# jiaxiZeng/Temporally-Consistent-Stereo-Matching

Hardware: AMD Instinct MI355X
Metric: stereo-pairs/sec at 640x480 D=192, 32 GRU iters (higher is better)
Workload: dtype f32

## Files before the change

### include/tcs_mi355.h

```cpp
#ifndef TCS_MI355_H
#define TCS_MI355_H

#include <stddef.h>
#include <stdint.h>

#ifdef __cplusplus
extern "C" {
#endif

#define TCS_OK 0
#define TCS_EINVAL (-1)
#define TCS_ELAUNCH (-2)
#define TCS_EUNSUPPORTED (-3)

typedef void* tcs_stream_t;

int tcs_abi_version(void);
const char* tcs_error_string(int code);


size_t tcs_corr_level_bytes(int B, int H, int W, int level);
size_t tcs_corr_build_workspace_bytes(int B, int H, int W);

int tcs_corr_build(const float* fmap1, const float* fmap2, int B, int C, int H, int W,
// ... 85 lines not shown
                      int B, int H, int W, float* refined, float* delta_disp, float* coords1, float* flow_x, float* flow_x_ch,
                      long long flow_x_ch_bstride, tcs_stream_t stream);

int tcs_convex_upsample(const float* disp, const float* mask, int B, int H, int W, int clip, float* flow_up, float* flow_q,
                        tcs_stream_t stream);

int tcs_convex_upsample_pair(const float* disp_a, const float* disp_b, const float* mask, int B, int H, int W, float* up_a, float* up_b,
                             float* q_a, float* q_b, tcs_stream_t stream);

int tcs_avgpool3s2(const float* x, int B, int C, int H, int W, float* out, tcs_stream_t stream);

int tcs_resize_bilinear(const float* x, int B, int C, int H, int W, int Ho, int Wo, float* out, tcs_stream_t stream);
int tcs_resize_bilinear_scaled(const float* x, int B, int C, int H, int W, int Ho, int Wo, float scale, float* out, tcs_stream_t stream);

#define TCS_ACT_NONE 0
#define TCS_ACT_RELU 1
#define TCS_ACT_SIGMOID 2
#define TCS_ACT_TANH 3
#define TCS_ACT_LEAKY 4
#define TCS_ACT_RELU_ADD_RELU 5

#define TCS_EPI_LINEAR 0
#define TCS_EPI_GRU_ZR 1
#define TCS_EPI_GRU_Q 2
#define TCS_EPI_BLEND9 4
#define TCS_EPI_DECONV2X 3

#define TCS_MATH_F32 0
#define TCS_MATH_F16X3 1

#define TCS_MAX_SRC 4

typedef struct tcs_conv_desc {
    const float* src[TCS_MAX_SRC];
    int src_ch[TCS_MAX_SRC];
    int n_src;
    const float* weight;
    const float* bias;
    int B, H, W;
    int Cin, Cout, ksize;
    int epilogue;
    int act;
    float post_scale;
    const float* addend;
    const float* addend2;
    const float* h;
    const float* z;
    int blend_keep_z;
    float* out;
    int out_ctot, out_coff;
    float* out2;
    int stride;
    int math;
    float weight_unscale;
    void* out16;
    int out16_groups, out16_group_offset;
    int in_transform;
    const float* src_batch2;
    int batch_split;
    int products;
} tcs_conv_desc;

size_t tcs_conv_packed_floats(int Cout, int Cin, int ksize);
int tcs_pack_conv_weight(const float* w_oihw, int Cout, int Cin, int ksize, float* packed, tcs_stream_t stream);
size_t tcs_conv_packed_floats_f16x3(int Cout, int Cin, int ksize);
int tcs_pack_conv_weight_f16x3(const float* w_oihw, int Cout, int Cin, int ksize, int scale_log2, float* packed,
                               tcs_stream_t stream);
size_t tcs_deconv_packed_floats_f16x3(int Cin, int Cout);
int tcs_pack_deconv4x4s2_f16x3(const float* w_iohw, int Cin, int Cout, int scale_log2, float* packed, float* scratch_oihw,
                               tcs_stream_t stream);
int tcs_instance_norm(const float* x, int B, int C, int H, int W, float eps, int act, const float* addend, float* out,
                      tcs_stream_t stream);
int tcs_conv3x3_cout1(const float* x, const float* w_oihw, const float* bias, int B, int Cin, int H, int W, float* out,
                      tcs_stream_t stream);
int tcs_conv2d(const tcs_conv_desc* desc, tcs_stream_t stream);
int tcs_conv2d_group(const tcs_conv_desc* const* descs, int n, tcs_stream_t stream);
int tcs_conv2d_group_fused(const tcs_conv_desc* const* descs, int n);

size_t tcs_s16_bytes(int B, int C, int H, int W);
int tcs_s16_flags(unsigned int* flags_out);
#define TCS_S16_FLAG_UNITS 5
int tcs_s16_flags_detail(unsigned int* per_unit);
int tcs_s16_from_f32(const float* x, int B, int C, int H, int W, void* s16, int groups_total, int group_offset, tcs_stream_t stream);
int tcs_s16_to_f32(const void* s16, int B, int C, int H, int W, int groups_total, int group_offset, float* out, tcs_stream_t stream);

typedef struct tcs_conv_s16_desc {
    const void* src[TCS_MAX_SRC];
    int src_ch[TCS_MAX_SRC];
    int src_groups[TCS_MAX_SRC];
    int n_src;
    const float* weight;
    const float* bias;
    int B, H, W;
    int Cin, Cout, ksize;
    int stride;
    int epilogue;
    int act;
    float post_scale;
    float weight_unscale;
    const float* addend;
    const float* addend2;
    const void* addend16;
    int addend16_groups;
    const void* h;
    int h_groups;
    const float* z;
    int blend_keep_z;
    void* out16;
    int out16_groups, out16_group_offset;
    float* out32;
    int out_ctot, out_coff;
    int tile_cfg;
    int addend_ctot;
    const float* blend_cand;
    int blend_cand_ctot;
    const float* blend_disp;
    float* blend_refined;
    float* blend_delta;
    float* blend_coords1;
    float* blend_flow_x;
    void* blend_flow16;
    int blend_flow16_groups, blend_flow16_channel;
    void* out16b;
    int out16b_groups, out16_split;
    void* in_stats;
    float in_eps;
    const float* tap_weights;
    float* tap_out;
    int tap_nout, tap_tiles;
    float tap_unscale;
    const float* blend_warm_pyr[4];
    int blend_warm_radius;
    int products;
} tcs_conv_s16_desc;

int tcs_avgpool3s2_s16(const void* x, int B, int groups, int H, int W, void* out, int out_groups, tcs_stream_t stream);
int tcs_resize_bilinear_s16(const void* x, int B, int groups, int H, int W, int Ho, int Wo, void* out, int out_groups, tcs_stream_t stream);
size_t tcs_instance_norm_s16_workspace_bytes(int B, int groups, int H, int W);
int tcs_instance_norm_s16(const void* x, int B, int groups, int H, int W, float eps, int act, const void* addend, int addend_groups,
                          void* out, int out_groups, void* workspace, tcs_stream_t stream);
size_t tcs_deconv_in_stats_bytes(int B, int C, int H_in, int W_in);
int tcs_instance_norm_apply_s16(const void* x, int B, int groups, int H, int W, int act, const void* addend, int addend_groups,
                                void* out, int out_groups, const void* in_stats, int C, float eps, tcs_stream_t stream);
size_t tcs_tap_weights_floats(int nout, int C);
int tcs_pack_tap_weights(const float* w_oihw, int nout, int C, int scale_log2, float* packed, tcs_stream_t stream);
int tcs_taps_sum(const float* taps, int ntile, int nout, const float* bias, const float* addend, float scale, int B, int H, int W, float* out,
                 tcs_stream_t stream);
int tcs_flow_taps_step_grads(const float* coords1, const float* taps, int ntile, const float* bias, int B, int H, int W, float scale,
                             float* disp_q, float* grad, float* cands, float* delta_out, tcs_stream_t stream);
int tcs_taps_propagate_s16(const float* taps, int ntile, const float* bias2, const float* g5, float post_scale, const float* disp, int B, int H,
                           int W, float* grad_out, float* cand9, void* out16, int out_groups, tcs_stream_t stream);
int tcs_propagate_disparity_s16(const float* grad, const float* disp, int B, int H, int W, float* cand9, void* out16, int out_groups,
                                tcs_stream_t stream);
int tcs_s16_set_channel(const float* x, int B, int H, int W, void* s16, int groups_total, int channel, tcs_stream_t stream);
int tcs_softmax_blend_s16(const float* logits9, const float* cand, int cand_ctot, const float* disp_q,
                          int B, int H, int W, float* refined, float* delta_disp, float* coords1, float* flow_x,
                          void* flow_x_s16, int flow_x_s16_groups, int flow_x_s16_channel, tcs_stream_t stream);

size_t tcs_weight_frags_bytes(int Cout, int Cin);
int tcs_pack_weight_frags(const float* w_oi, int Cout, int Cin, int natural_channels, int scale_log2, void* packed, tcs_stream_t stream);
int tcs_hidden_update_s16(void* h, int h_groups, const float* delta, const float* w1, const float* b1, const void* W2, const float* b2,
                          float unscale2, const void* Wzr, const float* bzr, float unscale_zr, const void* Wq, const float* bq,
                          float unscale_q, int B, int H, int W, tcs_stream_t stream);

int tcs_conv2d_s16(const tcs_conv_s16_desc* desc, tcs_stream_t stream);

int tcs_conv2d_s16_group(const tcs_conv_s16_desc* const* descs, int n, tcs_stream_t stream);
int tcs_conv2d_s16_group_fused(const tcs_conv_s16_desc* const* descs, int n);

typedef struct tcs_s16_instance { int ksize, stride, epilogue, mt, rows, ksteps, nstage, row_split, rows_per_wave, taps,
                                  products, csplit, blocks, threads; long long lds_bytes; } tcs_s16_instance;
int tcs_conv2d_s16_plan(const tcs_conv_s16_desc* desc, tcs_s16_instance* out);

#define TCS_LOSS_MAX_ITERS 64
#define TCS_LOSS_SEQ 1
#define TCS_LOSS_INIT 2
#define TCS_LOSS_GRAD 4
#define TCS_LOSS_NORM 8
#define TCS_LOSS_OUT_TOTAL 0
#define TCS_LOSS_OUT_SEQ 1
#define TCS_LOSS_OUT_INIT 2
#define TCS_LOSS_OUT_NORM 3
#define TCS_LOSS_OUT_GRAD 4
#define TCS_LOSS_OUT_EPE 5
#define TCS_LOSS_OUT_INIT_GT 14
#define TCS_LOSS_OUT_INIT_NM 15
#define TCS_LOSS_OUT_FMR 16
#define TCS_LOSS_OUT_FLAGS 17
#define TCS_LOSS_NOUT 18

size_t tcs_loss_workspace_bytes(int B, int H, int W, int iters);
int tcs_loss_targets(const float* flow_gt, const void* valid, int valid_mode, int B, int H, int W, float* grad_gt, float* norm_gt,
                     uint8_t* grad_mask, uint8_t* norm_mask, uint8_t* valid_dense, uint8_t* valid_sparse, tcs_stream_t stream);
int tcs_loss_targets_full(const float* gt, int C, const void* valid, int valid_mode, int B, int H, int W, float* out, uint8_t* gt_mask,
                          uint8_t* valid_dense, uint8_t* valid_sparse, tcs_stream_t stream);
int tcs_sequence_loss(const float* preds, long long iter_stride, long long refine_offset, int iters, const float* flow_gt,
                      const void* valid, int valid_mode, const float* flow_mono, const float* flow_init, int B, int H, int W,
                      double* workspace, tcs_stream_t stream);
int tcs_init_loss(const float* cost_volume, int D, const float* flow_gt, const void* valid, int valid_mode, int B, int H, int W, int k,
                  float threshold, int iters, double* workspace, tcs_stream_t stream);
int tcs_grad_normal_loss(const float* grad_preds, long long grad_stride, const float* q_preds, long long q_stride, long long q_refine_offset,
                         int iters, const float* grad_gt, const uint8_t* grad_mask, const uint8_t* grad_valid, const float* norm_gt,
                         const uint8_t* norm_mask, const uint8_t* norm_valid, int B, int H, int W, double* workspace, tcs_stream_t stream);
int tcs_loss_finish(const double* workspace, int parts, int B, int H, int W, int iters, int k, const double* loss_weights, double* out,
                    float* out32, tcs_stream_t stream);

#define TCS_LOSS_COUNT_SEQ 0
#define TCS_LOSS_COUNT_INIT 1
#define TCS_LOSS_COUNT_NORM 2
#define TCS_LOSS_COUNT_GRAD 3
#define TCS_LOSS_NCOUNTS 4
int tcs_loss_finish_counts(const double* workspace, int parts, int B, int H, int W, int iters, int k, const double* loss_weights,
                           double* out, float* out32, double* counts, tcs_stream_t stream);
int tcs_sequence_loss_bwd(const float* preds, long long iter_stride, long long refine_offset, int iters, const float* flow_gt,
                          const void* valid, int valid_mode, const float* flow_mono, const float* flow_init, int B, int H, int W,
                          const double* loss_weights, const double* counts, const float* upstream, float* grad_preds, float* grad_mono,
                          float* grad_init, tcs_stream_t stream);
int tcs_init_loss_bwd(const float* cost_volume, int D, const float* flow_gt, const void* valid, int valid_mode, int B, int H, int W, int k,
                      float threshold, const double* counts, const float* upstream, float* grad_cost_volume, tcs_stream_t stream);
int tcs_grad_normal_loss_bwd(const float* grad_preds, long long grad_stride, const float* q_preds, long long q_stride,
                             long long q_refine_offset, int iters, const float* grad_gt, const uint8_t* grad_mask, const uint8_t* grad_valid,
                             const float* norm_gt, const uint8_t* norm_mask, const uint8_t* norm_valid, int B, int H, int W,
                             const double* loss_weights, const double* counts, const float* upstream, float* grad_grad_preds,
                             float* grad_q_preds, tcs_stream_t stream);

int tcs_upsample_flow(const float* flow, const float* mask, int B, int H, int W, float* flow_up, tcs_stream_t stream);
int tcs_upsample_flow_pair(const float* flow_a, const float* flow_b, const float* mask, int B, int H, int W, float* up_a, float* up_b,
                           tcs_stream_t stream);
size_t tcs_convex_upsample_backward_workspace_floats(int B, int H, int W, int n_flows);
int tcs_convex_upsample_backward(const float* flow, const float* mask, const float* grad_up, int B, int H, int W, float* grad_mask,
                                 float* grad_flow, float* workspace, tcs_stream_t stream);
int tcs_convex_upsample_pair_backward(const float* flow_b, const float* mask, const float* grad_up_a, const float* grad_up_b, int B, int H,
                                      int W, float* grad_mask, float* grad_flow_a, float* grad_flow_b, float* workspace, tcs_stream_t stream);
int tcs_refine_blend(const float* logits9, const float* disp_grads, const float* disp, int B, int H, int W, float* refined,
                     tcs_stream_t stream);
int tcs_refine_blend_backward(const float* logits9, const float* disp_grads, const float* disp, const float* grad_refined, int B, int H,
                              int W, float* grad_logits, float* grad_disp_grads, tcs_stream_t stream);

#ifdef __cplusplus
}
#endif
#endif
```

### temporally-consistent-stereo-matching_amd/core/tc_stereo.py

```python
import contextlib
import os

import torch
import torch.nn as nn

from core.corr import CorrBlock1D
from core.extractor import BasicEncoder, MultiBasicEncoder, ResidualBlock, hip_head
from core.update import (IN_SUM_SLOTS, BasicMultiUpdateBlock, DispGradPredictor, DispRefine, DisparityCompletor, HiddenstateUpdater,
                         Lightfuse, hip_conv)
from core.utils.utils import coords_grid
from tcs_mi355 import ops, s16


class autocast(contextlib.AbstractContextManager):

    def __init__(self, enabled=False, **_):
        self.enabled = enabled

    def __exit__(self, *exc):
        return False


HIP_PRECISIONS = {"fp32": 0, "fp16": 1}

# ... 144 lines not shown
        if test_mode:
            return self._pipeline()(image1, image2, iters, temporal, use_graph=self._graph_mode())
        out = self._pipeline()(image1, image2, iters, temporal, use_graph=self._graph_mode(), outputs=True)
        return self._training_output(out, iters)

    @staticmethod
    def _training_output(out, iters):
        up, q, grad = out["up"], out["q"], out["grad"]
        return {"flow_mono": out["flow_mono"], "flow_init": out["flow_init"],
                "flow_predictions": [[up[k, 0], up[k, 1]] for k in range(iters)],
                "flow_q_predictions": [[q[k, 0], q[k, 1]] for k in range(iters)],
                "disp_grad_q_predictions": [grad[k] for k in range(iters)],
                "cost_volume": out["cost_volume"],
                "flow_q": out["flow_q"], "net_list": out["net_list"], "fmap1": out["fmap1"]}

    def _frame(self, image1, image2, iters, temporal, outputs=False):
        feats = self._extract_stage(image1, image2, temporal is None or len(temporal) == 8, outputs)
        return self._refine_loop(feats, self._refine_head(feats, temporal), iters, outputs)

    def _extract_stage(self, image1, image2, first, cost_volume=False):
        a = self.args

        def correlate(fmap1, fmap2):
            corr_fn = CorrBlock1D(fmap1, fmap2, radius=a.corr_radius, num_levels=a.corr_levels, thres=a.init_thres, want_argmax=first,
                                  want_cost_volume=cost_volume)
            return corr_fn, (corr_fn.argmax_disp() if first else None)

        def context(cnet_list, relu_done=False):
            inp = [x[1] if relu_done else torch.relu(x[1]) for x in cnet_list]
            grads = [hip_conv(conv, [i]) for i, conv in zip(inp, self.context_zqr_convs_grad)]
            zqr = [list(hip_conv(conv, [i]).chunk(3, 1)) for i, conv in zip(inp, self.context_zqr_convs)]
            return zqr, grads, [x[0] for x in cnet_list]

        if a.shared_backbone and self.cnet.can16(image1):
            from tcs_mi355.streams import fork_join
            trunk = self.cnet.trunk16(image1, right=image2, raw_images=True)

            def matching_side():
                fm = hip_head(self.conv2, trunk)
                f1, f2 = (t.float().contiguous() for t in fm.split(fm.shape[0] // 2, 0))
                return f1, f2, correlate(f1, f2)

            (fmap1, fmap2, (corr_fn, prior)), (inp_list, grad_list, net_list) = fork_join(
                [matching_side, lambda: context(self.cnet.heads16(trunk, True, a.n_gru_layers, relu_context=True), relu_done=True)])
        else:
            image1 = (2 * (image1 / 255.0) - 1.0).contiguous()
            image2 = (2 * (image2 / 255.0) - 1.0).contiguous()
            cnet_list, fmap1, fmap2 = self._features(image1, image2)
            corr_fn, prior = correlate(fmap1, fmap2)
            inp_list, grad_list, net_list = context(cnet_list)
        return {"fmap1": fmap1, "corr_fn": corr_fn, "prior": prior, "inp_list": inp_list, "grad_list": grad_list, "net_list": net_list}

    def _refine_head(self, feats, temporal):
        first = temporal is None
        start = temporal[7] if temporal is not None and len(temporal) == 8 else None
        fmap1, corr_fn = feats["fmap1"], feats["corr_fn"]
        net_list = feats["net_list"]
        if first:
            last_net_list = None
            sparse_disp, cost, sparse_mask = feats["prior"] if feats["prior"] is not None else corr_fn.argmax_disp()
        else:
            K, T, previous_T, baseline, last_disp, last_net_list, last_fmap1 = temporal[:7]
            K_scale, K_scale_inv, relative_T, back_T = ops.pose_prepare(K, T, previous_T, self.scale_rate, start=start)
            prior = None if start is None else (feats["prior"] if feats["prior"] is not None else corr_fn.argmax_disp())
            sparse_disp, _, sparse_mask, cost = ops.warp_forward(
                (-last_disp).float().contiguous(), last_fmap1.float().contiguous(), relative_T, K_scale,
                K_scale_inv, baseline, cur_fmap=fmap1, want_fmap=False, ordered=self._hip_deterministic, start=start, prior=prior)

        pool = self._s16pool
        disp_init, disp_mono, _, net_list = self.disp_completor.run16(pool, sparse_disp, cost, sparse_mask,
                                                                      [c.float().contiguous() for c in net_list], tanh_nets=True)
        disp_init = disp_init.float().contiguous()

        if last_net_list is None:
            warped = None
        else:
            grid = ops.backward_grid(disp_init, back_T, K_scale, K_scale_inv, baseline)
            warped = []
            for i, net in enumerate(last_net_list):
                warped.append(ops.bilinear_sample(net.float().contiguous(), grid, start=start))
                if i + 1 < len(last_net_list):
                    grid = ops.grid_halve(grid)

        for i, (h, fuse) in enumerate(zip(net_list, self.previous_current_hideen_fuse)):
            if warped is None:
                x = pool.get(("frame", "zero", i), h.B, h.C, h.H, h.W, h.device)
            else:
                x = s16.to_s16(warped[i], out=pool.get(("frame", "warped", i), h.B, h.C, h.H, h.W, h.device))
            fuse.step16(pool, h, [x])

        coords0 = self._coords0(fmap1)
        coords1 = (coords0 - disp_init).contiguous()
        trace = getattr(self, "_trace", None)
        if trace is not None:
            trace.update(sparse_disp=sparse_disp, cost=cost, sparse_mask=sparse_mask, disp_init=disp_init,
                         net0=[t.float().clone() for t in net_list], iters=[])
        return {"coords1": coords1, "net_list": net_list, "disp_init": disp_init, "disp_mono": disp_mono}

    def _refine_loop(self, feats, start, iters, outputs=False):
        a = self.args
        fmap1, corr_fn = feats["fmap1"], feats["corr_fn"]
        inp_list, grad_list = feats["inp_list"], feats["grad_list"]
        coords1, nets = start["coords1"], start["net_list"]
        coords0 = self._coords0(fmap1)
        trace = getattr(self, "_trace", None)

        pool = self._s16pool
        n3 = a.n_gru_layers == 3
        grads16 = [s16.to_s16(t.float().contiguous(), out=pool.get(("frame", "ctxg", i), t.shape[0], t.shape[1], t.shape[2], t.shape[3], t.device))
                   for i, t in enumerate(grad_list)]
        dg_pre = self.disp_grad_refine.prepare(pool, grads16)
        self.disp_grad_refine.begin_frame(pool, coords1.shape[0], coords1.device)
        refined = up_mask = None
        flows_x = (coords1 - coords0).contiguous()
        motion = pool.get(("frame", "motion"), coords1.shape[0], 128, coords1.shape[2], coords1.shape[3], coords1.device)
        s16.set_channel(flows_x, motion, 127)
        ub = self.update_block
        ub.begin_frame()
        from tcs_mi355.streams import fork_join, join, mark, spawn
        hu_delta = None
        early32 = None
        plain = not a.slow_fast_gru and n3
        side = _OutputsSide(self, pool, coords1, iters, start) if outputs else None
        for itr in range(iters):
            def enc_branch():
                corr = corr_fn(coords1)
                return corr, ub.encoder.run(pool, flows_x, corr, motion)

            def coarse_branch():
                if hu_delta is not None:
                    self.hiddenstate_update.run(pool, nets[0], hu_delta)
                if up32_now is not None:
                    return ub.gru16_late(pool, nets, up32_now[1])
                if n3 and a.slow_fast_gru:
                    ub.run_coarse(pool, nets, inp_list, iter16=False, iter32=True, want_up16=False)
                if a.n_gru_layers >= 2 and a.slow_fast_gru:
                    ub.run_coarse(pool, nets, inp_list, iter16=True, iter32=n3, want_up16=False)
                return ub.run_coarse(pool, nets, inp_list, iter16=a.n_gru_layers >= 2, iter32=n3, up32=up32_now)

            up32_now = join(early32)
            early32 = None
            up16, (corr, m) = fork_join([coarse_branch, enc_branch])
            if side is not None:
                side.launch()
            run_ahead = plain and trace is None and itr + 1 < iters
            def ahead():
                up32 = ub.run_gru32(pool, nets, inp_list)
                return up32, ub.gru16_early(pool, nets, inp_list, up32)
            at_join = mark() if run_ahead else None
            sums = getattr(self, "_checksums", None)
            lazy = trace is None and sums is None
            delta_flow = ub.run_fine(pool, nets, inp_list, m, up16, lazy=lazy)
            if at_join is not None:
                early32 = spawn(ahead, after=at_join)
            if isinstance(delta_flow, s16.Taps):
                disp_q, g5, cands = s16.flow_taps_step_grads(coords1, delta_flow, scale=5.0)
            else:
                disp_q, g5, cands = ops.flow_step_grads(coords1, delta_flow, scale=5.0)
            disp_grad, context = self.disp_grad_refine.run(pool, g5, cands, dg_pre, lazy=lazy, slot=itr if itr < IN_SUM_SLOTS else None)
            last = itr == iters - 1
            warm = corr_fn._pyr if (not last and a.corr_levels == 4) else None
            if side is None:
                refined, up_mask, fused = self.disp_refine.run(pool, disp_grad, disp_q, nets[0], context, want_mask=last, motion=motion,
                                                               warm_pyramid=warm, warm_radius=a.corr_radius)
            else:
                refined, up_mask, fused = self.disp_refine.run(pool, disp_grad, disp_q, nets[0], context, motion=motion,
                                                               warm_pyramid=warm, warm_radius=a.corr_radius, grad_out=side.grad[itr],
                                                               before_fuse=side.join)
                side.record(itr, disp_q, refined, fused["fused"])
            hu_delta = fused["delta_disp"]
            coords1, flows_x = fused["coords1"], fused["flow_x"]
            if sums is not None:
                sums.append({k: v.double().sum() for k, v in dict(
                    corr=corr, motion=m.data, net0=nets[0].data, net1=nets[1].data, net2=nets[2].data, delta_flow=delta_flow,
                    disp_grad=disp_grad, context=context.data, refined=refined, coords1=coords1).items()})
            if trace is not None:
                self.hiddenstate_update.run(pool, nets[0], hu_delta)
                hu_delta = None
                trace["iters"].append(dict(corr=corr, delta=delta_flow, disp_q=disp_q, refined=refined,
                                           net=[t.float() for t in nets]))
        if hu_delta is not None:
            self.hiddenstate_update.run(pool, nets[0], hu_delta)
        if side is not None:
            side.launch()
            up_mask = side.join()
        net_list = [t.float() for t in nets]

        flow_up, flow_q = ops.convex_upsample(refined.contiguous(), up_mask)
        out = {"flow": flow_up, "flow_q": flow_q, "net_list": [x.detach() for x in net_list], "fmap1": fmap1.detach()}
        if side is not None:
            out.update(side.outputs(corr_fn))
        return out

# ... 52 lines not shown
```

### temporally-consistent-stereo-matching_amd/core/update.py

```python
import torch
import torch.nn as nn
import torch.nn.functional as F

from core.utils.basic_layers import Conv2x_IN
from tcs_mi355 import ops, s16
from tcs_mi355.streams import fork_join


CONV_MATH = "f16x3"


def products_of(conv: nn.Module) -> int:
    if getattr(conv, "_tcs_x3", False):
        return 0
    pool = getattr(conv, "_s16pool", None)
    return 0 if pool is None else pool.products


def packed(conv: nn.Conv2d) -> ops.PackedConv:
    w, b = conv.weight, conv.bias
    math = getattr(conv, "_tcs_math", None) or CONV_MATH
    if conv.stride == (2, 2):
        math = "f16x3"
    nprod = products_of(conv) if math == "f16x3" else 0
# ... 21 lines not shown


def packed16_part(conv: nn.Conv2d, cin_slices, with_bias: bool = True) -> ops.PackedConv:
    w, b = conv.weight, conv.bias
    nprod = products_of(conv)
    key = (w.data_ptr(), w._version, w.device, None if b is None else (b.data_ptr(), b._version), nprod)
    cache = conv.__dict__.setdefault("_tcs_parts", {})
    spec = (tuple(tuple(int(v) for v in sl) for sl in cin_slices), bool(with_bias))
    hit = cache.get(spec)
    if hit is None or hit[0] != key:
        ws = torch.cat([w.detach()[:, lo:hi] for lo, hi in spec[0]], 1).contiguous()
        hit = (key, ops.pack_conv(ws, b if with_bias else None, "f16x3", nprod))
        cache[spec] = hit
    return hit[1]


def packed16_cat(convs) -> ops.PackedConv:
    nprod = products_of(convs[0])
    key = tuple((c.weight.data_ptr(), c.weight._version, None if c.bias is None else (c.bias.data_ptr(), c.bias._version)) for c in convs) + (nprod,)
    host = convs[0]
    cache = host.__dict__.setdefault("_tcs_cat", {})
    ids = tuple(id(c) for c in convs)
    hit = cache.get(ids)
    if hit is None or hit[0] != key:
        w = torch.cat([c.weight.detach() for c in convs], 0).contiguous()
        b = torch.cat([(c.bias.detach() if c.bias is not None else torch.zeros(c.out_channels, device=c.weight.device)) for c in convs], 0).contiguous()
        hit = (key, ops.pack_conv(w, b, "f16x3", nprod))
        cache[ids] = hit
    return hit[1]


def tap_weights(conv2: nn.Conv2d) -> torch.Tensor:
    w = conv2.weight
    key = (w.data_ptr(), w._version, w.device)
    hit = getattr(conv2, "_tcs_taps", None)
    if hit is None or hit[0] != key:
        hit = (key, s16.pack_taps(w))
        conv2._tcs_taps = hit
    return hit[1]


def tap_partials(pool, conv1: nn.Conv2d, conv2: nn.Conv2d, srcs, pc=None, out16b=None) -> s16.Taps:
    a = srcs[0]
    ntile = (conv1.out_channels + 31) // 32
    taps = s16.Taps(pool.get32((id(conv2), "taps"), (a.B, ntile, 9 * conv2.out_channels, a.H, a.W), a.device), ntile, conv2.out_channels,
                    None if conv2.bias is None else conv2.bias.detach())
    s16.conv2d(packed16(conv1) if pc is None else pc, srcs, act="relu", taps=taps, tap_weights=tap_weights(conv2), out16b=out16b,
               out16_split=conv1.out_channels if out16b is not None else 0)
    return taps


def pool_of(module) -> s16.S16Pool:
    p = getattr(module, "_s16pool", None)
    if p is None:
        p = s16.S16Pool()
        for m in module.modules():
            m._s16pool = p
    return p


def conv16(pool, conv, srcs, act="none", addend=None, post_scale=1.0, out=None, want32=False, tag="o", addend16=None, pc=None, tile_cfg=0):
    a = srcs[0]
    pc = packed16(conv) if pc is None else pc
    stride = conv.stride[0]
    Ho, Wo = ((a.H - 1) // 2 + 1, (a.W - 1) // 2 + 1) if stride == 2 else (a.H, a.W)
    if want32:
        return s16.conv2d(pc, srcs, act=act, addend=addend, post_scale=post_scale, want32=True, stride=stride, addend16=addend16)[1]
    if out is None:
        out = pool.get((id(conv), tag), a.B, conv.out_channels, Ho, Wo, a.device)
    return s16.conv2d(pc, srcs, act=act, addend=addend, post_scale=post_scale, out16=out, stride=stride, addend16=addend16, tile_cfg=tile_cfg)[0]


def conv32to16(pool, conv, x, act="none", tag="o", image_pair=None, in_transform=0):
    B, _, H, W = (int(v) for v in x.shape)
    B += 0 if image_pair is None else int(image_pair.shape[0])
    out = pool.get((id(conv), tag), B, conv.out_channels, H, W, x.device)
    return ops.conv2d(packed(conv), [x.float().contiguous()], act=act, out16=out,
                      image_pair=None if image_pair is None else image_pair.float().contiguous(), in_transform=in_transform)


def to16(pool, x, key):
    B, C_, H, W = (int(v) for v in x.shape)
    return s16.to_s16(x.float().contiguous(), out=pool.get(key, B, C_, H, W, x.device))


IN_SUM_SLOTS = 64


def up_block16(pool, block: Conv2x_IN, x: s16.S16, rem: s16.S16, slot=None) -> s16.S16:
    dc = block.conv1.conv
    y = pool.get((id(dc), "o"), x.B, dc.out_channels, 2 * x.H, 2 * x.W, x.device)
    stats = None
    if slot is not None and s16.deconv_in_stats_ok(x.B, dc.out_channels, x.H, x.W):
        stats = up_block_sums(pool, block, x.B, x.device)[int(slot)]
    s16.deconv4x4s2(packed_deconv(dc), [x], out16=y, in_stats=stats)
    norm = (lambda **kw: s16.instance_norm_apply(y, stats, **kw)) if stats is not None else (lambda **kw: s16.instance_norm(y, **kw))
    if (y.H, y.W) != (rem.H, rem.W):
        y32 = F.interpolate(norm(act="leaky", out=y).float(), size=(rem.H, rem.W), mode="nearest") + rem.float()
        y = to16(pool, y32, (id(dc), "resized"))
    else:
        y = norm(act="leaky", addend=rem, out=y)
    act2 = "leaky" if block.conv2.relu else "none"
    if block.conv2.use_in:
        z = conv16(pool, block.conv2.conv, [y])
        return s16.instance_norm(z, act=act2, out=z)
    return conv16(pool, block.conv2.conv, [y], act=act2)


def up_block_sums(pool, block: Conv2x_IN, B: int, device) -> torch.Tensor:
    dc = block.conv1.conv
    stride = s16.nv.lib().tcs_deconv_in_stats_bytes(1, dc.out_channels, 8, 8) // (8 * dc.out_channels)
    return pool.get_i64((id(dc), "in_sums"), (IN_SUM_SLOTS, int(B), dc.out_channels, stride), device)


def hip_conv(conv, srcs, act="none", **kw):
    return ops.conv2d(packed(conv), [s.float().contiguous() for s in srcs], act=act, stride=conv.stride[0], **kw)


def packed_deconv(deconv: nn.ConvTranspose2d) -> ops.PackedConv:
    w = deconv.weight
    nprod = products_of(deconv)
    key = (w.data_ptr(), w._version, w.device, nprod)
    hit = getattr(deconv, "_tcs_packed", None)
    if hit is None or hit[0] != key:
        if deconv.kernel_size != (4, 4) or deconv.stride != (2, 2) or deconv.padding != (1, 1) or deconv.bias is not None:
            raise NotImplementedError(f"tcs deconv covers ConvTranspose2d(4, stride 2, pad 1, bias=False), got {deconv}")
        hit = (key, ops.pack_deconv4x4s2(w, nprod))
        deconv._tcs_packed = hit
    return hit[1]


def _conv(cin, cout, k, stride=1):
    return nn.Conv2d(cin, cout, k, stride, k // 2)


def _two(cin, mid, cout, k=3, tail=None):
    layers = [_conv(cin, mid, k), nn.ReLU(inplace=True), _conv(mid, cout, k)]
    return nn.Sequential(*layers, *([tail] if tail is not None else []))


class _GateCell(nn.Module):
    keep_z = False

    def __init__(self, hidden_dim, input_dim, kernel_size):
        super().__init__()
        self.convzr = _conv(hidden_dim + input_dim, hidden_dim * 2, kernel_size)
        self.convq = _conv(hidden_dim + input_dim, hidden_dim, kernel_size)

    def _step(self, h, xs, cz=None, cr=None, cq=None):
        h = h.float().contiguous()
        xs = [x.float().contiguous() for x in xs]
        z, rh = ops.gru_gates(packed(self.convzr), [h, *xs], h, cz, cr)
        return ops.gru_update(packed(self.convq), [rh, *xs], h, z, cq, keep_z=self.keep_z)

    def step16(self, pool, h: s16.S16, xs, cz=None, cr=None, cq=None) -> s16.S16:
        z = pool.get32((id(self), "z"), (h.B, h.C, h.H, h.W), h.device)
        rh = pool.get((id(self), "rh"), h.B, h.C, h.H, h.W, h.device)
        ctot = lambda t: 0 if (t is None or t.is_contiguous()) else int(t.stride(0)) // (h.H * h.W)
        if ctot(cz) != ctot(cr):
            cz, cr = cz.contiguous(), cr.contiguous()
        s16.gru_gates(packed16(self.convzr), [h, *xs], h, cz, cr, z_out=z, rh_out=rh, addend_ctot=ctot(cz))
        return s16.gru_update(packed16(self.convq), [rh, *xs], h, z, cq, keep_z=self.keep_z, out=h, addend_ctot=ctot(cq))


class ConvGRU(_GateCell):
    def __init__(self, hidden_dim, input_dim, kernel_size=3):
# ... 305 lines not shown

    def propagate_disparity(self, disparity_grad, disparity_map):
        buf = ops.propagate_disparity(disparity_grad.float().contiguous(), disparity_map.float().contiguous())
        return buf[:, :9], buf[:, 9:]

    def forward(self, disp_grads, disp, context_disp, context_grad, test_mode=False, fused_outputs=None):
        pool = pool_of(self)
        cd = to16(pool, context_disp, (id(self), "ctxd_in"))
        cg = to16(pool, context_grad, (id(self), "ctxg_in"))
        refined, mask, extra = self.run(pool, disp_grads.float().contiguous(), disp.float().contiguous(), cd, cg, want_mask=not test_mode)
        if fused_outputs is not None:
            fused_outputs.update({k: v for k, v in extra.items() if k != "fused"})
        return refined, mask

    def mask_head(self, pool, fused: s16.S16, out: torch.Tensor = None) -> torch.Tensor:
        m = conv16(pool, self.mask[0], [fused], act="relu")
        if out is None:
            return conv16(pool, self.mask[2], [m], post_scale=0.25, want32=True)
        return s16.conv2d(packed16(self.mask[2]), [m], post_scale=0.25, out32=out)[1]

    def run(self, pool, disp_grads: torch.Tensor, disp: torch.Tensor, context_disp: s16.S16, context_grad: s16.S16, want_mask=False,
            motion: s16.S16 = None, warm_pyramid=None, warm_radius: int = 4, grad_out: torch.Tensor = None, before_fuse=None):
        f27 = pool.get((id(self), "f27"), disp.shape[0], 27, disp.shape[2], disp.shape[3], disp.device)
        if isinstance(disp_grads, tuple):
            f27, cand9, self._last_grad = s16.taps_propagate(disp_grads[0], disp_grads[1], disp_grads[2], disp, out16=f27, grad=grad_out)
        else:
            f27, cand9 = s16.propagate_disparity(disp_grads, disp, out16=f27)
            if grad_out is not None:
                grad_out.copy_(disp_grads)

        cc, ds = self.context_compress, self.disp_f_stem
        t3 = 101411 if context_disp.H * context_disp.W >= 10000 else 0
        with s16.grouped():
            c = conv16(pool, cc[0], [context_disp, context_grad], act="relu", tile_cfg=t3)
            d = conv16(pool, ds[0], [f27], act="relu")
        with s16.grouped():
            context = conv16(pool, cc[2], [c], tile_cfg=t3)
            disp_f = conv16(pool, ds[2], [d])
        fused = conv16(pool, self.conv_fuse[0], [disp_f, context], act="relu")
        if before_fuse is not None:
            before_fuse()
        fused = conv16(pool, self.conv_fuse[2], [fused], act="relu")
        w = conv16(pool, self.w_head[0], [fused], act="relu")
        coords1, flow_x = torch.empty_like(disp), torch.empty_like(disp)
        refined, delta = s16.conv1x1_blend(packed16(self.w_head[2]), [w], cand9, disp, coords1, flow_x, flow_x_s16=motion,
                                           flow_x_channel=127, warm_pyramid=warm_pyramid, warm_radius=warm_radius)
        mask = self.mask_head(pool, fused) if want_mask else None
        return refined, mask, dict(delta_disp=delta, coords1=coords1, flow_x=flow_x, fused=fused)


class DisparityCompletor(nn.Module):
    def __init__(self):
        super().__init__()
        relu = lambda: nn.ReLU(inplace=True)
        mlp = lambda cin, mid, cout: nn.Sequential(_conv(cin, mid, 1), relu(), _conv(mid, cout, 1))
        cin_block = lambda cin, mid, cout, s=1: nn.Sequential(_conv(cin, mid, 3, s), nn.InstanceNorm2d(mid), relu(), _conv(mid, cout, 3))
        self.conv_disp_stem = mlp(1, 64, 64)
        self.conv_cost_stem = mlp(1, 32, 32)
        self.conv_mask_stem = mlp(1, 32, 32)
        self.conv_disp_fuse = mlp(128, 128, 64)
        self.conv_4_4 = cin_block(192, 192, 64)
        self.conv_4_8 = cin_block(64, 64, 64, 2)
        self.conv_8_8 = cin_block(192, 192, 64)
        self.conv_8_16 = cin_block(64, 64, 64, 2)
        self.conv_16_16 = cin_block(192, 192, 64)
        self.conv_16_8 = Conv2x_IN(64, 64, deconv=True, concat=False, keep_concat=False, IN=True)
        self.conv_8_4 = Conv2x_IN(64, 64, deconv=True, concat=False, keep_concat=False, IN=True)
        self.disp_head = _two(64, 128, 1)
        self.w_head = _two(64, 128, 1, tail=nn.Sigmoid())
        self.conv_out16_disp = cin_block(192, 192, 128)
        self.conv_out8_disp = cin_block(192, 192, 128)
        self.conv_out4_disp = cin_block(192, 192, 128)

    def run16(self, pool, disp, cost, mask, ctx, tanh_nets=False):
        d = (disp / 10).float().contiguous()

        def stem(seq, x):
            return conv16(pool, seq[2], [conv32to16(pool, seq[0], x.float().contiguous(), act="relu")])

        def cin(seq, srcs, act="none"):
            y = conv16(pool, seq[0], srcs)
            return conv16(pool, seq[3], [s16.instance_norm(y, act="relu", out=y)], act=act)

        c16 = [to16(pool, c, (id(self), "ctx", i)) for i, c in enumerate(ctx)]
        x4_disp = conv16(pool, self.conv_disp_fuse[2], [conv16(pool, self.conv_disp_fuse[0], [stem(self.conv_disp_stem, d),
                         stem(self.conv_cost_stem, cost), stem(self.conv_mask_stem, mask - 0.5)], act="relu")])
        x4 = cin(self.conv_4_4, [x4_disp, c16[0]])
        x8 = cin(self.conv_8_8, [cin(self.conv_4_8, [x4]), c16[1]])
        x16_out = cin(self.conv_16_16, [cin(self.conv_8_16, [x8]), c16[2]])
        x8_out = up_block16(pool, self.conv_16_8, x16_out, x8)
        x4_out = up_block16(pool, self.conv_8_4, x8_out, x4)
        disp_mono = conv16(pool, self.disp_head[2], [conv16(pool, self.disp_head[0], [x4_out], act="relu")], want32=True)
        w = conv16(pool, self.w_head[2], [conv16(pool, self.w_head[0], [x4_out], act="relu")], act="sigmoid", want32=True)
        completed = (w * d + (1 - w) * disp_mono) * 10
        na = "tanh" if tanh_nets else "none"
        nets = [cin(self.conv_out4_disp, [x4_out, c16[0]], na), cin(self.conv_out8_disp, [x8_out, c16[1]], na),
                cin(self.conv_out16_disp, [x16_out, c16[2]], na)]
        return completed, disp_mono * 10, w, nets

    def forward(self, disp, cost, mask, context_list, tanh_nets=False):
        if not disp.is_cuda:
            raise RuntimeError("DisparityCompletor: CPU tensor (the hot path has no CPU fallback)")
        completed, mono, w, nets = self.run16(pool_of(self), disp, cost, mask, [c.float().contiguous() for c in context_list], tanh_nets)
        return completed, mono, w, [n.float() for n in nets]
```

### temporally-consistent-stereo-matching_amd/csrc/tcs_conv_s16.hip

```cpp
#include "tcs_conv_common.h"
#include "tcs_s16.h"

typedef float float4_t __attribute__((ext_vector_type(4)));

struct S16Args {
    const _Float16* src[TCS_MAX_SRC];
    int src_groups[TCS_MAX_SRC];
    int src_kend[TCS_MAX_SRC];
    const float* w;
    const float* bias;
    int B, H, W;
    int Hin, Win;
    int nk;
    int Cout, nct32;
    int act;
    float post_scale, w_unscale;
    const float* add1;
    const float* add2;
    int add_ctot;
    const _Float16* add16;
    int add16_groups;
    const _Float16* h;
    int h_groups;
    const float* z;
// ... 451 lines not shown
        const unsigned addr_b = addr_b0 + (unsigned)buf * STAGE_BYTES, addr_a = addr_a0 + (unsigned)buf * STAGE_BYTES;
        Frag f0, f1;
        S16_FETCH(f0, 0)
#pragma unroll
        for (int i = 0; i < NSTEP; i += 2) {
            if (i + 1 < NSTEP) { S16_FETCH(f1, (i + 1 < NSTEP ? i + 1 : 0)) S16_WAIT_LGKM(R) } else S16_WAIT_LGKM(0)
            S16_MMA(f0)
            if (i + 1 < NSTEP) {
                if (i + 2 < NSTEP) { S16_FETCH(f0, (i + 2 < NSTEP ? i + 2 : 0)) S16_WAIT_LGKM(R) } else S16_WAIT_LGKM(0)
                S16_MMA(f1)
            }
        }
        if (NSTAGE == 1 && s + 1 < nstage_total) {
            __builtin_amdgcn_s_barrier();
            S16_ISSUE(0, s + 1)
        }
        buf = buf + 1 == NSTAGE ? 0 : buf + 1;
    }
#undef S16_ISSUE
#undef S16_FETCH
#undef S16_MMA

    const int px = x0 + l31, py = y0 + wave * RPW;
    if constexpr (EPI == TCS_EPI_DECONV2X) {
        if (a.in_ws) {
            extern __shared__ __attribute__((aligned(16))) float s16_dyn_lds[];
            s16_deconv_sums<MT, ROWS>(a, b, ct, py, px, wave, lane, acc, s16_dyn_lds);
        }
    }
#pragma unroll
    for (int j = 0; j < RPW; ++j) {
        if (TP) {
            const bool st = px < a.W && py + j < a.H;
#pragma unroll
            for (int m = 0; m < MT; ++m)
                s16_epilogue_tile<EPI, true>(a, b, (ct * MT + m) * 32 + 4 * half, min(py + j, a.H - 1), min(px, a.W - 1), acc[m * RPW + j], st);
        } else if (px < a.W && py + j < a.H) {
#pragma unroll
            for (int m = 0; m < MT; ++m) s16_epilogue_tile<EPI>(a, b, (ct * MT + m) * 32 + 4 * half, py + j, px, acc[m * RPW + j]);
        }
    }
}

template <int KS, int MT, int ROWS, int KSTEPS, int NSTAGE, int STRIDE, int EPI, int RS = 0, int RPW = 1, bool TP = false>
__global__ __launch_bounds__(64 * ROWS / RPW, s16_min_waves(MT, EPI, RPW, TP)) void k_conv_s16(S16Args a) {
    s16_conv_body<KS, MT, ROWS, KSTEPS, NSTAGE, STRIDE, EPI, RS, RPW, TP>(a, blockIdx.x, gridDim.x, blockIdx.y);
}

template <int KS, int MT, int ROWS, int KSTEPS, int NSTAGE, int STRIDE, int EPI, int RS = 0, int RPW = 1, bool TP = false>
__global__ __launch_bounds__(64 * ROWS / RPW, s16_min_waves(MT, EPI, RPW, TP)) void k_conv_s16_x1(S16Args a) {
    s16_conv_body<KS, MT, ROWS, KSTEPS, NSTAGE, STRIDE, EPI, RS, RPW, TP, 1>(a, blockIdx.x, gridDim.x, blockIdx.y);
}

template <int KS0, int MT0, int ROWS0, int KST0, int NST0, int EPI0, int KS1, int MT1, int ROWS1, int KST1, int NST1, int EPI1>
__global__ __launch_bounds__(64 * (ROWS0 > ROWS1 ? ROWS0 : ROWS1),
                             (s16_min_waves(MT0, EPI0, 1, false) < s16_min_waves(MT1, EPI1, 1, false) ? s16_min_waves(MT0, EPI0, 1, false)
                                                                                                      : s16_min_waves(MT1, EPI1, 1, false)))
void k_conv_s16_pair(S16Args a0, S16Args a1, int n0, int n0pad) {
    const int bid = blockIdx.x;
    if (bid < n0pad) {
        if (bid >= n0 || (int)threadIdx.x >= 64 * ROWS0) return;
        s16_conv_body<KS0, MT0, ROWS0, KST0, NST0, 1, EPI0>(a0, bid, n0, blockIdx.y);
    } else {
        if ((int)threadIdx.x >= 64 * ROWS1) return;
        s16_conv_body<KS1, MT1, ROWS1, KST1, NST1, 1, EPI1>(a1, bid - n0pad, (int)gridDim.x - n0pad, blockIdx.y);
    }
}

template <int KS0, int MT0, int ROWS0, int KST0, int NST0, int EPI0, int KS1, int MT1, int ROWS1, int KST1, int NST1, int EPI1>
__global__ __launch_bounds__(64 * (ROWS0 > ROWS1 ? ROWS0 : ROWS1),
                             (s16_min_waves(MT0, EPI0, 1, false) < s16_min_waves(MT1, EPI1, 1, false) ? s16_min_waves(MT0, EPI0, 1, false)
                                                                                                      : s16_min_waves(MT1, EPI1, 1, false)))
void k_conv_s16_x1_pair(S16Args a0, S16Args a1, int n0, int n0pad) {
    const int bid = blockIdx.x;
    if (bid < n0pad) {
        if (bid >= n0 || (int)threadIdx.x >= 64 * ROWS0) return;
        s16_conv_body<KS0, MT0, ROWS0, KST0, NST0, 1, EPI0, 0, 1, false, 1>(a0, bid, n0, blockIdx.y);
    } else {
        if ((int)threadIdx.x >= 64 * ROWS1) return;
        s16_conv_body<KS1, MT1, ROWS1, KST1, NST1, 1, EPI1, 0, 1, false, 1>(a1, bid - n0pad, (int)gridDim.x - n0pad, blockIdx.y);
    }
}

__global__ __launch_bounds__(256) void k_s16_from_f32(const float* __restrict__ x, int C, int H, int W, int G, int goff, int Gtot,
                                                       _Float16* __restrict__ out) {
    const int HW = H * W;
    const size_t n = (size_t)G * HW;
    const size_t i = (size_t)blockIdx.x * 256 + threadIdx.x;
    const int b = blockIdx.y;
    if (i >= n) return;
    const int g = (int)(i / HW), p = (int)(i - (size_t)g * HW);
    const int y = p / W, xx = p - y * W;
    float v[8];
#pragma unroll
    for (int j = 0; j < 8; ++j) {
        const int c = g * 8 + j;
        v[j] = c < C ? x[((size_t)b * C + c) * HW + p] : 0.f;
    }
    half4 h0, l0, h1, l1;
    split4(v, h0, l0);
    split4(v + 4, h1, l1);
    half8 hi, lo;
#pragma unroll
    for (int j = 0; j < 4; ++j) { hi[j] = h0[j]; hi[j + 4] = h1[j]; lo[j] = l0[j]; lo[j + 4] = l1[j]; }
    _Float16* o = out + s16_unit(b, Gtot, goff + g, 0, H + 2, W + 2, y, xx);
    *reinterpret_cast<half8*>(o) = hi;
    *reinterpret_cast<half8*>(o + (size_t)(H + 2) * (W + 2) * 8) = lo;
}

__global__ __launch_bounds__(256) void k_s16_to_f32(const _Float16* __restrict__ s, int C, int H, int W, int Gtot, int goff,
                                                     float* __restrict__ out) {
    const int HW = H * W, G = (C + 7) / 8;
    const size_t n = (size_t)G * HW;
    const size_t i = (size_t)blockIdx.x * 256 + threadIdx.x;
    const int b = blockIdx.y;
    if (i >= n) return;
    const int g = (int)(i / HW), p = (int)(i - (size_t)g * HW);
    const int y = p / W, xx = p - y * W;
    const _Float16* u = s + s16_unit(b, Gtot, goff + g, 0, H + 2, W + 2, y, xx);
    const half8 hi = *reinterpret_cast<const half8*>(u);
    const half8 lo = *reinterpret_cast<const half8*>(u + (size_t)(H + 2) * (W + 2) * 8);
#pragma unroll
    for (int j = 0; j < 8; ++j) {
        const int c = g * 8 + j;
        if (c < C) out[((size_t)b * C + c) * HW + p] = (float)hi[j] + (float)lo[j];
    }
}

struct S16Plan {
    bool filled;
    long long key;
    int nprod;
    S16Args args;
    int nblocks, threads, B;
    size_t lds;
    int (*launch_alone)(S16Args&, hipStream_t);
};
static thread_local S16Plan* g_s16_plan = nullptr;

constexpr long long s16_key(int KS, int MT, int ROWS, int KSTEPS, int NSTAGE, int STRIDE, int EPI, int RS, int RPW, bool TP) {
    return ((((((((((long long)KS * 10 + MT) * 10 + ROWS) * 10 + KSTEPS) * 10 + NSTAGE) * 10 + STRIDE) * 10 + EPI) * 10 + RS) * 10 + RPW) * 2 + (TP ? 1 : 0));
}

template <int KS, int MT, int ROWS, int KSTEPS, int NSTAGE, int STRIDE, int EPI, int RS = 0, int RPW = 1, bool TP = false, int NPR = 3>
static int launch_s16(S16Args& a, hipStream_t s) {
    constexpr bool GATHER = KS == 1 && STRIDE == 2;
    constexpr int IH = RS ? ROWS : (GATHER ? ROWS : STRIDE * ROWS + KS - STRIDE), IW = GATHER ? 32 : STRIDE * 32 + KS - STRIDE, TS = RS ? KS : KS * KS;
    constexpr int NPL = NPR == 3 ? 2 : 1;
    constexpr int NPI = (KSTEPS * 2 * NPL * IH * IW + 63) / 64, NP = NPI + KSTEPS * TS * MT * NPL;
    constexpr size_t lds = (size_t)NSTAGE * NP * 1024;
    static_assert(lds <= 160 * 1024, "LDS budget");
    auto kern = NPR == 3 ? k_conv_s16<KS, MT, ROWS, KSTEPS, NSTAGE, STRIDE, EPI, RS, RPW, TP>
                         : k_conv_s16_x1<KS, MT, ROWS, KSTEPS, NSTAGE, STRIDE, EPI, RS, RPW, TP>;
    a.npx = tcs_cdiv(a.W, 32);
    a.nct = a.nct32 / MT;
    a.npatch = a.npx * tcs_cdiv(a.H, ROWS);
    if (a.csplit > 0 && a.nct % a.csplit != 0) a.csplit = 1;
    if (g_s16_plan && !g_s16_plan->filled) {
        S16Plan& p = *g_s16_plan;
        p.filled = true;
        p.key = s16_key(KS, MT, ROWS, KSTEPS, NSTAGE, STRIDE, EPI, RS, RPW, TP);
        p.nprod = NPR;
        p.args = a;
        p.nblocks = a.npatch * a.nct; p.threads = 64 * ROWS / RPW; p.B = a.B; p.lds = lds;
        p.launch_alone = &launch_s16<KS, MT, ROWS, KSTEPS, NSTAGE, STRIDE, EPI, RS, RPW, TP, NPR>;
        return TCS_OK;
    }
    (void)hipGetLastError();
    if (lds > 64 * 1024) {
        if (hipFuncSetAttribute(reinterpret_cast<const void*>(kern), hipFuncAttributeMaxDynamicSharedMemorySize, (int)lds) != hipSuccess)
            return TCS_ELAUNCH;
    }
    hipLaunchKernelGGL(kern, dim3(a.npatch * a.nct, a.B), dim3(64 * ROWS / RPW), lds, s, a);
    return tcs_launch_status();
}

template <int KS0, int MT0, int ROWS0, int KST0, int NST0, int EPI0, int KS1, int MT1, int ROWS1, int KST1, int NST1, int EPI1, int NPR>
static int launch_s16_pair(const S16Plan& p0, const S16Plan& p1, hipStream_t s) {
    auto kern = NPR == 3 ? k_conv_s16_pair<KS0, MT0, ROWS0, KST0, NST0, EPI0, KS1, MT1, ROWS1, KST1, NST1, EPI1>
                         : k_conv_s16_x1_pair<KS0, MT0, ROWS0, KST0, NST0, EPI0, KS1, MT1, ROWS1, KST1, NST1, EPI1>;
    const size_t lds = p0.lds > p1.lds ? p0.lds : p1.lds;
    (void)hipGetLastError();
    if (lds > 64 * 1024) {
        if (hipFuncSetAttribute(reinterpret_cast<const void*>(kern), hipFuncAttributeMaxDynamicSharedMemorySize, (int)lds) != hipSuccess)
            return TCS_ELAUNCH;
    }
    const int n0pad = (p0.nblocks + 7) & ~7;
    hipLaunchKernelGGL(kern, dim3(n0pad + p1.nblocks, p0.B), dim3(64 * (ROWS0 > ROWS1 ? ROWS0 : ROWS1)), lds, s, p0.args, p1.args, p0.nblocks, n0pad);
    return tcs_launch_status();
}
// ... 53 lines not shown
#undef S16_CASE
#undef S16_CASE_RS
#undef S16_CASE_RPW2
}

static int s16_heuristic(const S16Args& a, int ksize, int stride, int kst1x1, int epilogue) {
    if (ksize == 1 && stride == 2) return 100000 + 1000 + 400 + 10 + 2;
    if (ksize == 1) {
        const int mt = (a.nct32 % 2 == 0 && a.nct32 >= 8) ? 2 : 1;
        return 100000 + mt * 1000 + 400 + kst1x1 * 10 + 2;
    }
    if (stride == 2) {
        const long long blocks4 = (long long)tcs_cdiv(a.W, 32) * tcs_cdiv(a.H, 4) * a.B * a.nct32;
        return blocks4 > 256 ? 101411 : 101412;
    }
    const long long blocks8 = (long long)tcs_cdiv(a.W, 32) * tcs_cdiv(a.H, 8) * a.B * a.nct32;
    if (blocks8 >= 280) {
        if (a.nct32 >= 8 && a.nk >= 16) return 100000 + 1000 + 800 + 10 + 2;
        return 100000 + 1000 + 400 + 10 + 1;
    }
    if (blocks8 >= 180) return 100000 + 1000 + 800 + 10 + 2;
    return 100000 + 1000 + 400 + 10 + 2;
}

template <int NPR>
static int s16_launch_epi(const tcs_conv_s16_desc* d, S16Args& a, int cfg, int stride, hipStream_t s) {
    switch (d->epilogue) {
        case TCS_EPI_LINEAR:
            if (stride == 2 && d->ksize == 1) return launch_s16_cfg<1, 2, TCS_EPI_LINEAR, NPR>(a, cfg, s);
            if (stride == 2) return launch_s16_cfg<3, 2, TCS_EPI_LINEAR, NPR>(a, cfg, s);
            return d->ksize == 3 ? launch_s16_cfg<3, 1, TCS_EPI_LINEAR, NPR>(a, cfg, s) : launch_s16_cfg<1, 1, TCS_EPI_LINEAR, NPR>(a, cfg, s);
        case TCS_EPI_BLEND9:
            if (d->ksize != 1 || stride != 1 || d->Cout != 9 || !d->blend_cand || d->blend_cand_ctot < 9 || !d->blend_refined) return TCS_EINVAL;
            if (d->blend_delta && !d->blend_disp) return TCS_EINVAL;
            if (d->blend_flow16 && (d->blend_flow16_channel < 0 || d->blend_flow16_channel >= 8 * d->blend_flow16_groups)) return TCS_EINVAL;
            a.bl_cand = d->blend_cand; a.bl_cand_ctot = d->blend_cand_ctot; a.bl_disp = d->blend_disp;
            a.bl_refined = d->blend_refined; a.bl_delta = d->blend_delta; a.bl_coords1 = d->blend_coords1; a.bl_flow = d->blend_flow_x;
            a.bl_f16 = reinterpret_cast<_Float16*>(d->blend_flow16); a.bl_f16_groups = d->blend_flow16_groups; a.bl_f16_ch = d->blend_flow16_channel;
            if (d->blend_warm_pyr[0]) {
                if (!d->blend_warm_pyr[1] || !d->blend_warm_pyr[2] || !d->blend_warm_pyr[3] || d->blend_warm_radius < 0 || d->blend_warm_radius > 16 ||
                    d->W < 8) return TCS_EINVAL;
                a.warm_pyr0 = d->blend_warm_pyr[0]; a.warm_pyr1 = d->blend_warm_pyr[1]; a.warm_pyr2 = d->blend_warm_pyr[2];
                a.warm_pyr3 = d->blend_warm_pyr[3]; a.warm_radius = d->blend_warm_radius;
            }
            return launch_s16_cfg<1, 1, TCS_EPI_BLEND9, NPR>(a, cfg, s);
        case TCS_EPI_DECONV2X:
            if (d->ksize != 3 || !a.out16 || d->Cout % 32 != 0) return TCS_EINVAL;
            a.hidden = d->Cout / 4;
            return launch_s16_cfg<3, 1, TCS_EPI_DECONV2X, NPR>(a, cfg, s);
        case TCS_EPI_GRU_ZR:
            if (!a.h || !a.out16 || !a.out32 || d->Cout % 64 != 0) return TCS_EINVAL;
            a.hidden = d->Cout / 2;
            if (a.h_groups < a.hidden / 8) return TCS_EINVAL;
            return d->ksize == 3 ? launch_s16_cfg<3, 1, TCS_EPI_GRU_ZR, NPR>(a, cfg, s) : launch_s16_cfg<1, 1, TCS_EPI_GRU_ZR, NPR>(a, cfg, s);
        case TCS_EPI_GRU_Q:
            if (!a.h || !a.z || !a.out16 || d->Cout % 32 != 0) return TCS_EINVAL;
            a.hidden = d->Cout;
            if (a.h_groups < a.hidden / 8) return TCS_EINVAL;
            return d->ksize == 3 ? launch_s16_cfg<3, 1, TCS_EPI_GRU_Q, NPR>(a, cfg, s) : launch_s16_cfg<1, 1, TCS_EPI_GRU_Q, NPR>(a, cfg, s);
        default: return TCS_EINVAL;
    }
}

extern "C" {

size_t tcs_deconv_in_stats_bytes(int B, int C, int H, int W) {
    if (B <= 0 || C <= 0 || C % 32 != 0 || H <= 0 || W <= 0 || (long long)4 * H * W > (1 << 20)) return 0;
    return (size_t)B * C * S16_IN_STRIDE * sizeof(long long);
}

size_t tcs_s16_bytes(int B, int C, int H, int W) {
    if (B <= 0 || C <= 0 || H <= 0 || W <= 0) return 0;
    const size_t G = (size_t)((C + 15) / 16) * 2;
    return (size_t)B * G * 2 * (H + 2) * (W + 2) * 16;
}

int tcs_s16_from_f32(const float* x, int B, int C, int H, int W, void* s16, int groups_total, int group_offset, tcs_stream_t stream) {
    if (!x || !s16 || B <= 0 || B > 65535 || C <= 0 || H <= 0 || W <= 0) return TCS_EINVAL;
    const int G = ((C + 15) / 16) * 2;
    if (group_offset < 0 || (group_offset & 1) || group_offset + G > groups_total) return TCS_EINVAL;
    const size_t n = (size_t)G * H * W;
    hipLaunchKernelGGL(k_s16_from_f32, dim3((unsigned)((n + 255) / 256), B), dim3(256), 0, tcs_stream(stream), x, C, H, W, G, group_offset,
                       groups_total, reinterpret_cast<_Float16*>(s16));
    return tcs_launch_status();
}

int tcs_s16_to_f32(const void* s16, int B, int C, int H, int W, int groups_total, int group_offset, float* out, tcs_stream_t stream) {
    if (!out || !s16 || B <= 0 || B > 65535 || C <= 0 || H <= 0 || W <= 0) return TCS_EINVAL;
    const int G = (C + 7) / 8;
    if (group_offset < 0 || group_offset + G > groups_total) return TCS_EINVAL;
    const size_t n = (size_t)G * H * W;
    hipLaunchKernelGGL(k_s16_to_f32, dim3((unsigned)((n + 255) / 256), B), dim3(256), 0, tcs_stream(stream),
                       reinterpret_cast<const _Float16*>(s16), C, H, W, groups_total, group_offset, out);
    return tcs_launch_status();
}

int tcs_conv2d_s16(const tcs_conv_s16_desc* d, tcs_stream_t stream) {
    if (!d || !d->weight || d->n_src < 1 || d->n_src > TCS_MAX_SRC) return TCS_EINVAL;
    if (d->B <= 0 || d->B > 65535 || d->H <= 0 || d->W <= 0 || d->Cout <= 0) return TCS_EINVAL;
    if (d->ksize != 1 && d->ksize != 3) return TCS_EUNSUPPORTED;
    const int nprod = d->products == 0 ? 3 : d->products;
    if (nprod != 1 && nprod != 3) return TCS_EINVAL;
    const int stride = d->stride == 2 ? 2 : 1;
    if (stride == 2 && d->epilogue != TCS_EPI_LINEAR) return TCS_EUNSUPPORTED;
    S16Args a;
    int ktot = 0, cin = 0;
    for (int i = 0; i < TCS_MAX_SRC; ++i) {
        const bool used = i < d->n_src;
        if (used) {
            if (!d->src[i] || d->src_ch[i] <= 0 || d->src_groups[i] < ((d->src_ch[i] + 15) / 16) * 2 || (d->src_groups[i] & 1)) return TCS_EINVAL;
            if (i + 1 < d->n_src && d->src_ch[i] % 16 != 0) return TCS_EINVAL;
            const int k = (d->src_ch[i] + 15) / 16;
            ktot += k;
            cin += d->src_ch[i];
        }
        a.src[i] = reinterpret_cast<const _Float16*>(used ? d->src[i] : d->src[0]);
        a.src_groups[i] = used ? d->src_groups[i] : d->src_groups[0];
        a.src_kend[i] = used ? ktot : 0x7fffffff;
    }
    if (cin != d->Cin) return TCS_EINVAL;
    a.w = d->weight; a.bias = d->bias;
    a.B = d->B; a.Hin = d->H; a.Win = d->W;
    a.H = stride == 2 ? (d->H - 1) / 2 + 1 : d->H;
    a.W = stride == 2 ? (d->W - 1) / 2 + 1 : d->W;
    a.Cout = d->Cout; a.nct32 = (d->Cout + 31) / 32;
    a.act = d->act; a.post_scale = d->post_scale; a.w_unscale = d->weight_unscale;
    a.add1 = d->addend; a.add2 = d->addend2;
    a.add16 = reinterpret_cast<const _Float16*>(d->addend16); a.add16_groups = d->addend16_groups;
    if (a.add16 && (d->epilogue != TCS_EPI_LINEAR || a.add16_groups < (d->Cout + 7) / 8)) return TCS_EINVAL;
    if (d->act == TCS_ACT_RELU_ADD_RELU && !a.add16 && !a.add1) return TCS_EINVAL;
    a.h = reinterpret_cast<const _Float16*>(d->h); a.h_groups = d->h_groups; a.z = d->z;
    a.keep_z = d->blend_keep_z; a.hidden = 0;
    a.out16 = reinterpret_cast<_Float16*>(d->out16); a.out16_groups = d->out16_groups; a.out16_goff = d->out16_group_offset;
    a.out32 = d->out32; a.out_ctot = d->out_ctot; a.out_coff = d->out_coff;
    a.out16b = reinterpret_cast<_Float16*>(d->out16b); a.out16b_groups = d->out16b_groups; a.out16_split = d->out16_split;
    a.tap_w = d->tap_weights; a.tap_out = d->tap_out; a.tap_nout = d->tap_nout; a.tap_ntile = d->tap_tiles; a.tap_unscale = d->tap_unscale;
    if (a.tap_out) {
        if (d->epilogue != TCS_EPI_LINEAR || stride != 1 || !a.tap_w || a.tap_nout < 1 || a.tap_nout > 2 || a.tap_ntile < 1 ||
            a.tap_ntile > (d->Cout + 31) / 32) return TCS_EINVAL;
    }
    if (a.out16b) {
        if (d->epilogue != TCS_EPI_LINEAR || (!a.out16 && !a.tap_out) || a.out16_split <= 0 || a.out16_split % 32 != 0 || a.out16_split >= d->Cout) return TCS_EINVAL;
        if (a.out16b_groups < (d->Cout - a.out16_split + 7) / 8) return TCS_EINVAL;
    }
    a.in_ws = d->in_stats;
    if (a.in_ws && (d->epilogue != TCS_EPI_DECONV2X || d->Cout % 128 != 0 || (long long)4 * d->H * d->W > (1 << 20))) return TCS_EINVAL;
    a.npx = 0; a.nct = 0; a.npatch = 0;
    a.csplit = (d->tile_cfg / 100000) % 10;
    a.bl_cand = nullptr; a.bl_cand_ctot = 0; a.bl_disp = nullptr; a.bl_refined = nullptr; a.bl_delta = nullptr; a.bl_coords1 = nullptr;
    a.bl_flow = nullptr; a.bl_f16 = nullptr; a.bl_f16_groups = 0; a.bl_f16_ch = 0;
    a.warm_pyr0 = a.warm_pyr1 = a.warm_pyr2 = a.warm_pyr3 = nullptr; a.warm_radius = 0;
    if (!a.out16 && !a.out32 && !a.tap_out && d->epilogue != TCS_EPI_BLEND9) return TCS_EINVAL;
    const int kpack = ((d->Cin + 63) / 64) * 4;
    int kst = 1;
    if (d->ksize == 1) {
        kst = 2;
        for (int i = 0; i < d->n_src; ++i)
            if (((d->src_ch[i] + 15) / 16) % 2 != 0) kst = 1;
    }
    int cfg = d->tile_cfg % 100000;
    if (cfg) kst = (cfg / 10) % 10;
    if (kst != 1 && kst != 2 && kst != 4) return TCS_EINVAL;
    for (int i = 0; i < d->n_src; ++i)
        if (((d->src_ch[i] + 15) / 16) % kst != 0) {
            if (i + 1 == d->n_src && d->src_groups[i] >= 2 * (((d->src_ch[i] + 15) / 16 + kst - 1) / kst * kst)) {
                const int k = (d->src_ch[i] + 15) / 16, kp = (k + kst - 1) / kst * kst;
// ... 129 lines not shown
```

### temporally-consistent-stereo-matching_amd/csrc/tcs_stencil.hip

```cpp
#include "tcs_s16.h"

__global__ __launch_bounds__(256) void k_flow_step(float* __restrict__ coords1, const float* __restrict__ delta, int W, int n,
                                                   float* __restrict__ disp_q) {
    const int i = blockIdx.x * 256 + threadIdx.x;
    if (i >= n) return;
    const float c = coords1[i] + delta[i];
    coords1[i] = c;
    disp_q[i] = (float)(i % W) - c;
}

__global__ __launch_bounds__(256) void k_grad_xy(const float* __restrict__ disp, int H, int W, float scale, float* __restrict__ grad) {
    const int b = blockIdx.y, HW = H * W;
    const int p = blockIdx.x * 256 + threadIdx.x;
    if (p >= HW) return;
    const int y = p / W, x = p - y * W;
    const float* d = disp + (size_t)b * HW;
    const float c = d[p];
    const float r = d[y * W + min(x + 1, W - 1)];
    const float dn = d[min(y + 1, H - 1) * W + x];
    grad[((size_t)b * 2 + 0) * HW + p] = scale * (r - c);
    grad[((size_t)b * 2 + 1) * HW + p] = scale * (dn - c);
}

__global__ __launch_bounds__(256) void k_grad_candidates(const float* __restrict__ disp, int H, int W, float* __restrict__ out) {
// ... 466 lines not shown
#pragma unroll
    for (int k = 0; k < 9; ++k) { w[k] = expf(w[k] - m); s += w[k]; }
    float r = 0.f;
#pragma unroll
    for (int k = 0; k < 9; ++k) r = __builtin_fmaf(w[k] / s, c[k], r);
    refined[(size_t)b * HW + p] = r;
}

#define RB_TX 32
#define RB_TY 8
#define RB_SX (RB_TX + 2)
#define RB_SY (RB_TY + 2)
__global__ __launch_bounds__(256) void k_refine_blend_bwd(const float* __restrict__ logits, const float* __restrict__ grad,
                                                          const float* __restrict__ disp, const float* __restrict__ g, int H, int W,
                                                          float* __restrict__ dlogits, float* __restrict__ dgrad) {
    __shared__ float st[9][RB_SY * RB_SX];
    const int b = blockIdx.z, HW = H * W;
    const int tx0 = blockIdx.x * RB_TX, ty0 = blockIdx.y * RB_TY;
    const float* d = disp + (size_t)b * HW;
    const float* gx = grad + (size_t)b * 2 * HW;
    const float* gy = gx + HW;
    for (int e = threadIdx.x; e < RB_SY * RB_SX; e += 256) {
        const int ey = e / RB_SX, ex = e - ey * RB_SX;
        const int cy = ty0 + ey - 1, cx = tx0 + ex - 1;
        float t[9];
#pragma unroll
        for (int k = 0; k < 9; ++k) t[k] = 0.f;
        if (cy >= 0 && cy < H && cx >= 0 && cx < W) {
            const int p = cy * W + cx;
            const float* l = logits + (size_t)b * 9 * HW + p;
            float w[9], m = -INFINITY;
#pragma unroll
            for (int k = 0; k < 9; ++k) { w[k] = l[(size_t)k * HW]; m = fmaxf(m, w[k]); }
            float s = 0.f;
#pragma unroll
            for (int k = 0; k < 9; ++k) { w[k] = expf(w[k] - m); s += w[k]; }
            const float gg = g[(size_t)b * HW + p];
#pragma unroll
            for (int k = 0; k < 9; ++k) { w[k] = w[k] / s; t[k] = w[k] * gg; }
            if (dlogits && ey >= 1 && ey <= RB_TY && ex >= 1 && ex <= RB_TX) {
                float c[9];
                double r = 0.0;
#pragma unroll
                for (int v = 0; v < 3; ++v) {
#pragma unroll
                    for (int u = 0; u < 3; ++u) {
                        const int yy = cy + v - 1, xx = cx + u - 1;
                        const bool in = yy >= 0 && yy < H && xx >= 0 && xx < W;
                        const int q = min(max(yy, 0), H - 1) * W + min(max(xx, 0), W - 1);
                        const float dn = d[q];
                        const float gnx = in ? gx[q] : 0.f;
                        const float gny = in ? gy[q] : 0.f;
                        c[3 * v + u] = dn + gnx * (float)(1 - u) + gny * (float)(1 - v);
                    }
                }
#pragma unroll
                for (int k = 0; k < 9; ++k) r += (double)w[k] * (double)c[k];
#pragma unroll
                for (int k = 0; k < 9; ++k) dlogits[((size_t)b * 9 + k) * HW + p] = w[k] * (float)((double)c[k] - r) * gg;
            }
        }
#pragma unroll
        for (int k = 0; k < 9; ++k) st[k][e] = t[k];
    }
    if (!dgrad) return;
    __syncthreads();
    const int ly = threadIdx.x / RB_TX, lx = threadIdx.x - ly * RB_TX;
    const int y = ty0 + ly, x = tx0 + lx;
    if (y >= H || x >= W) return;
    float ax = 0.f, ay = 0.f;
#pragma unroll
    for (int v = 0; v < 3; ++v) {
#pragma unroll
        for (int u = 0; u < 3; ++u) {
            const float t = st[3 * v + u][(ly + 2 - v) * RB_SX + (lx + 2 - u)];
            ax += t * (float)(1 - u);
            ay += t * (float)(1 - v);
        }
    }
    dgrad[((size_t)b * 2 + 0) * HW + y * W + x] = ax;
    dgrad[((size_t)b * 2 + 1) * HW + y * W + x] = ay;
}

extern "C" {

size_t tcs_tap_weights_floats(int nout, int C) {
    if (nout < 1 || nout > 2 || C <= 0) return 0;
    return (size_t)((C + 31) / 32) * 2 * 128 * 4;
}

int tcs_pack_tap_weights(const float* w_oihw, int nout, int C, int scale_log2, float* packed, tcs_stream_t stream) {
    if (!w_oihw || !packed || nout < 1 || nout > 2 || C <= 0 || scale_log2 < -60 || scale_log2 > 60) return TCS_EINVAL;
    const int nk = ((C + 31) / 32) * 2, n = nk * 128;
    hipLaunchKernelGGL(k_pack_tap_weights, dim3((n + 255) / 256), dim3(256), 0, tcs_stream(stream), w_oihw, nout, C, nk, ldexpf(1.0f, scale_log2),
                       reinterpret_cast<uint4*>(packed));
    return tcs_launch_status();
}

int tcs_taps_sum(const float* taps, int ntile, int nout, const float* bias, const float* addend, float scale, int B, int H, int W, float* out,
                 tcs_stream_t stream) {
    if (!taps || !out || ntile <= 0 || nout < 1 || nout > 2 || B <= 0 || B > 65535 || H <= 0 || W <= 0) return TCS_EINVAL;
    auto kern = ntile == 8 ? k_taps_sum<8> : (ntile == 4 ? k_taps_sum<4> : k_taps_sum<0>);
    hipLaunchKernelGGL(kern, dim3(tcs_cdiv((long long)H * W, 256), B), dim3(256), 0, tcs_stream(stream), taps, ntile, nout, bias, addend,
                       scale, H, W, out);
    return tcs_launch_status();
}

int tcs_flow_taps_step_grads(const float* coords1, const float* taps, int ntile, const float* bias, int B, int H, int W, float scale,
                             float* disp_q, float* grad, float* cands, float* delta_out, tcs_stream_t stream) {
    if (!coords1 || !taps || !disp_q || !grad || !cands || ntile <= 0 || B <= 0 || B > 65535 || H <= 0 || W <= 0) return TCS_EINVAL;
    auto kern = ntile == 8 ? k_flow_taps_step_grads<8> : (ntile == 4 ? k_flow_taps_step_grads<4> : k_flow_taps_step_grads<0>);
    hipLaunchKernelGGL(kern, dim3(tcs_cdiv(W, FT_T), tcs_cdiv(H, FT_TY), B), dim3(256), 0, tcs_stream(stream), coords1, taps,
                       ntile, bias, H, W, scale, disp_q, grad, cands, delta_out);
    return tcs_launch_status();
}


int tcs_flow_step(float* coords1, const float* delta, int B, int H, int W, float* disp_q, tcs_stream_t stream) {
    if (!coords1 || !delta || !disp_q || B <= 0 || H <= 0 || W <= 0) return TCS_EINVAL;
    const int n = B * H * W;
    hipLaunchKernelGGL(k_flow_step, dim3(tcs_cdiv(n, 256)), dim3(256), 0, tcs_stream(stream), coords1, delta, W, n, disp_q);
    return tcs_launch_status();
}

int tcs_flow_step_grads(const float* coords1, const float* delta, int B, int H, int W, float scale, float* disp_q, float* grad,
                        float* cands, tcs_stream_t stream) {
    if (!coords1 || !delta || !disp_q || !grad || !cands || B <= 0 || B > 65535 || H <= 0 || W <= 0) return TCS_EINVAL;
    hipLaunchKernelGGL(k_flow_step_grads, dim3(tcs_cdiv((long long)H * W, 256), B), dim3(256), 0, tcs_stream(stream), coords1, delta, H, W,
                       scale, disp_q, grad, cands);
    return tcs_launch_status();
}

int tcs_disp_gradient_xy(const float* disp, int B, int H, int W, float scale, float* grad, tcs_stream_t stream) {
    if (!disp || !grad || B <= 0 || B > 65535 || H <= 0 || W <= 0) return TCS_EINVAL;
    hipLaunchKernelGGL(k_grad_xy, dim3(tcs_cdiv((long long)H * W, 256), B), dim3(256), 0, tcs_stream(stream), disp, H, W, scale, grad);
    return tcs_launch_status();
}

int tcs_grad_candidates(const float* disp, int B, int H, int W, float* cands, tcs_stream_t stream) {
    if (!disp || !cands || B <= 0 || B > 65535 || H <= 0 || W <= 0) return TCS_EINVAL;
    hipLaunchKernelGGL(k_grad_candidates, dim3(tcs_cdiv((long long)H * W, 256), B), dim3(256), 0, tcs_stream(stream), disp, H, W, cands);
    return tcs_launch_status();
}

int tcs_propagate_disparity(const float* grad, const float* disp, int B, int H, int W, float* out27, tcs_stream_t stream) {
    if (!grad || !disp || !out27 || B <= 0 || B > 65535 || H <= 0 || W <= 0) return TCS_EINVAL;
    hipLaunchKernelGGL(k_propagate, dim3(tcs_cdiv((long long)H * W, 256), B), dim3(256), 0, tcs_stream(stream), grad, disp, H, W, out27);
    return tcs_launch_status();
}

int tcs_softmax_blend(const float* logits9, const float* cand, int cand_ctot, const float* disp_q,
                      int B, int H, int W, float* refined, float* delta_disp, float* coords1, float* flow_x, float* flow_x_ch,
                      long long flow_x_ch_bstride, tcs_stream_t stream) {
    if (!logits9 || !cand || !refined || cand_ctot < 9 || B <= 0 || B > 65535 || H <= 0 || W <= 0) return TCS_EINVAL;
    if (delta_disp && !disp_q) return TCS_EINVAL;
    if (flow_x_ch && flow_x_ch_bstride < (long long)H * W) return TCS_EINVAL;
    hipLaunchKernelGGL(k_softmax_blend, dim3(tcs_cdiv((long long)H * W, 256), B), dim3(256), 0, tcs_stream(stream),
                       logits9, cand, cand_ctot, disp_q, W, H * W, refined, delta_disp, coords1, flow_x, flow_x_ch, flow_x_ch_bstride,
                       (_Float16*)nullptr, 0, 0, H);
    return tcs_launch_status();
}

int tcs_softmax_blend_s16(const float* logits9, const float* cand, int cand_ctot, const float* disp_q,
                          int B, int H, int W, float* refined, float* delta_disp, float* coords1, float* flow_x,
                          void* flow_x_s16, int flow_x_s16_groups, int flow_x_s16_channel, tcs_stream_t stream) {
    if (!logits9 || !cand || !refined || cand_ctot < 9 || B <= 0 || B > 65535 || H <= 0 || W <= 0) return TCS_EINVAL;
// ... 15 lines not shown

int tcs_convex_upsample_pair(const float* disp_a, const float* disp_b, const float* mask, int B, int H, int W, float* up_a, float* up_b,
                             float* q_a, float* q_b, tcs_stream_t stream) {
    if (!disp_a || !disp_b || !mask || !up_a || !up_b || !q_a || !q_b || B <= 0 || B > 65535 || H <= 0 || W <= 0) return TCS_EINVAL;
    if ((long long)16 * H * W > 0x7fffffffLL) return TCS_EUNSUPPORTED;
    hipLaunchKernelGGL(k_convex_upsample_pair<false>, dim3(tcs_cdiv((long long)16 * H * W, 256), B), dim3(256), 0, tcs_stream(stream),
                       disp_a, disp_b, mask, H, W, up_a, up_b, q_a, q_b);
    return tcs_launch_status();
}

int tcs_avgpool3s2(const float* x, int B, int C, int H, int W, float* out, tcs_stream_t stream) {
    if (!x || !out || B <= 0 || C <= 0 || H <= 0 || W <= 0) return TCS_EINVAL;
    if ((long long)B * C > 65535) return TCS_EUNSUPPORTED;
    const int Ho = (H - 1) / 2 + 1, Wo = (W - 1) / 2 + 1;
    hipLaunchKernelGGL(k_avgpool3s2, dim3(tcs_cdiv((long long)Ho * Wo, 256), B * C), dim3(256), 0, tcs_stream(stream), x, H, W, Ho, Wo, out);
    return tcs_launch_status();
}

static bool tcs_up_shape_ok(int B, int H, int W) { return B > 0 && B <= 65535 && H > 0 && W > 0 && (long long)16 * H * W <= 0x7fffffffLL; }

int tcs_upsample_flow(const float* flow, const float* mask, int B, int H, int W, float* flow_up, tcs_stream_t stream) {
    if (!flow || !mask || !flow_up || B <= 0 || H <= 0 || W <= 0) return TCS_EINVAL;
    if (!tcs_up_shape_ok(B, H, W)) return TCS_EUNSUPPORTED;
    hipLaunchKernelGGL(k_convex_upsample<true>, dim3(tcs_cdiv((long long)16 * H * W, 256), B), dim3(256), 0, tcs_stream(stream),
                       flow, mask, H, W, 0, flow_up, (float*)nullptr);
    return tcs_launch_status();
}

int tcs_upsample_flow_pair(const float* flow_a, const float* flow_b, const float* mask, int B, int H, int W, float* up_a, float* up_b,
                           tcs_stream_t stream) {
    if (!flow_a || !flow_b || !mask || !up_a || !up_b || B <= 0 || H <= 0 || W <= 0) return TCS_EINVAL;
    if (!tcs_up_shape_ok(B, H, W)) return TCS_EUNSUPPORTED;
    hipLaunchKernelGGL(k_convex_upsample_pair<true>, dim3(tcs_cdiv((long long)16 * H * W, 256), B), dim3(256), 0, tcs_stream(stream),
                       flow_a, flow_b, mask, H, W, up_a, up_b, (float*)nullptr, (float*)nullptr);
    return tcs_launch_status();
}

size_t tcs_convex_upsample_backward_workspace_floats(int B, int H, int W, int n_flows) {
    if (B <= 0 || H <= 0 || W <= 0 || n_flows < 0 || n_flows > 2) return 0;
    return (size_t)n_flows * 9 * B * H * W;
}

int tcs_convex_upsample_pair_backward(const float* flow_b, const float* mask, const float* grad_up_a, const float* grad_up_b, int B, int H,
                                      int W, float* grad_mask, float* grad_flow_a, float* grad_flow_b, float* workspace, tcs_stream_t stream) {
    if (!mask || B <= 0 || H <= 0 || W <= 0 || (!grad_mask && !grad_flow_a && !grad_flow_b)) return TCS_EINVAL;
    if ((grad_mask && (!flow_b || !grad_up_b)) || (grad_flow_a && !grad_up_a) || (grad_flow_b && !grad_up_b)) return TCS_EINVAL;
    if ((grad_flow_a || grad_flow_b) && !workspace) return TCS_EINVAL;
    if (((uintptr_t)grad_up_a | (uintptr_t)grad_up_b) & 15) return TCS_EINVAL;
    if (!tcs_up_shape_ok(B, H, W)) return TCS_EUNSUPPORTED;
    const size_t plane = (size_t)9 * B * H * W;
    float* ws_a = grad_flow_a ? workspace : nullptr;
    float* ws_b = grad_flow_b ? workspace + (grad_flow_a ? plane : 0) : nullptr;
    hipLaunchKernelGGL(k_upsample_flow_bwd, dim3(tcs_cdiv((long long)H * W, 64), B), dim3(256), 0, tcs_stream(stream), flow_b, mask,
                       grad_flow_a ? grad_up_a : nullptr, (grad_mask || grad_flow_b) ? grad_up_b : nullptr, H, W, grad_mask, ws_a, ws_b);
    if (grad_flow_a || grad_flow_b)
        hipLaunchKernelGGL(k_upsample_flow_bwd_gather, dim3(tcs_cdiv((long long)H * W, 256), B, 2), dim3(256), 0, tcs_stream(stream),
                           ws_a, ws_b, H, W, grad_flow_a, grad_flow_b);
    return tcs_launch_status();
}

int tcs_convex_upsample_backward(const float* flow, const float* mask, const float* grad_up, int B, int H, int W, float* grad_mask,
                                 float* grad_flow, float* workspace, tcs_stream_t stream) {
    return tcs_convex_upsample_pair_backward(flow, mask, nullptr, grad_up, B, H, W, grad_mask, nullptr, grad_flow, workspace, stream);
}

int tcs_refine_blend(const float* logits9, const float* disp_grads, const float* disp, int B, int H, int W, float* refined,
                     tcs_stream_t stream) {
    if (!logits9 || !disp_grads || !disp || !refined || B <= 0 || B > 65535 || H <= 0 || W <= 0) return TCS_EINVAL;
    hipLaunchKernelGGL(k_refine_blend, dim3(tcs_cdiv((long long)H * W, 256), B), dim3(256), 0, tcs_stream(stream), logits9, disp_grads,
                       disp, H, W, refined);
    return tcs_launch_status();
}

int tcs_refine_blend_backward(const float* logits9, const float* disp_grads, const float* disp, const float* grad_refined, int B, int H,
                              int W, float* grad_logits, float* grad_disp_grads, tcs_stream_t stream) {
    if (!logits9 || !grad_refined || B <= 0 || B > 65535 || H <= 0 || W <= 0 || (!grad_logits && !grad_disp_grads)) return TCS_EINVAL;
    if (grad_logits && (!disp_grads || !disp)) return TCS_EINVAL;
    if (tcs_cdiv(H, RB_TY) > 65535) return TCS_EUNSUPPORTED;
    hipLaunchKernelGGL(k_refine_blend_bwd, dim3(tcs_cdiv(W, RB_TX), tcs_cdiv(H, RB_TY), B), dim3(256), 0, tcs_stream(stream), logits9,
                       disp_grads, disp, grad_refined, H, W, grad_logits, grad_disp_grads);
    return tcs_launch_status();
}

int tcs_abi_version(void) { return 17; }

const char* tcs_error_string(int code) {
    switch (code) {
        case TCS_OK: return "ok";
        case TCS_EINVAL: return "invalid argument";
        case TCS_ELAUNCH: return "HIP launch failed";
        case TCS_EUNSUPPORTED: return "unsupported shape";
        default: return "unknown error";
    }
}

}

int tcs_s16_flag_take_stencil(unsigned int* out) {
    unsigned int v = 0, zero = 0;
    if (hipMemcpyFromSymbol(&v, HIP_SYMBOL(TCS_S16_FLAG_VAR), sizeof(v)) != hipSuccess) return TCS_ELAUNCH;
    if (v && hipMemcpyToSymbol(HIP_SYMBOL(TCS_S16_FLAG_VAR), &zero, sizeof(zero)) != hipSuccess) return TCS_ELAUNCH;
    *out |= v;
    return TCS_OK;
}
```

### temporally-consistent-stereo-matching_amd/csrc/tcs_warp.hip

```cpp
#include "tcs_common.h"

struct Cam {
    float K[9], Ki[9], T[12], bf;
};

__device__ __forceinline__ Cam load_cam(const float* __restrict__ T_rel, const float* __restrict__ K,
                                        const float* __restrict__ K_inv, const float* __restrict__ baseline, int b) {
    Cam c;
#pragma unroll
    for (int i = 0; i < 9; ++i) { c.K[i] = K[b * 9 + i]; c.Ki[i] = K_inv[b * 9 + i]; }
#pragma unroll
    for (int i = 0; i < 12; ++i) c.T[i] = T_rel[b * 16 + i];
    c.bf = baseline[b] * c.K[0];
    return c;
}

__device__ __forceinline__ float fix_nonfinite(float v) { return isfinite(v) ? v : -1.0f; }

__device__ __forceinline__ void reproject(const Cam& c, float disp, float x, float y, float& zp, float& u, float& v) {
    const float depth = c.bf / fmaxf(disp, 0.001f);
    const float rx = c.Ki[0] * x + c.Ki[1] * y + c.Ki[2];
    const float ry = c.Ki[3] * x + c.Ki[4] * y + c.Ki[5];
    const float rz = c.Ki[6] * x + c.Ki[7] * y + c.Ki[8];
    const float px = depth * rx, py = depth * ry, pz = depth * rz;
// ... 9 lines not shown
__device__ __forceinline__ void warp_geometry_body(const float* __restrict__ disp, const float* __restrict__ T_rel,
                                                   const float* __restrict__ K, const float* __restrict__ K_inv,
                                                   const float* __restrict__ baseline, const unsigned char* __restrict__ start,
                                                   int H, int W, float* __restrict__ cur_disp, float* __restrict__ valid,
                                                   float* __restrict__ flow, float* __restrict__ partial) {
    __shared__ float red[4];
    const int b = blockIdx.y, HW = H * W;
    const int p = blockIdx.x * 256 + threadIdx.x;
    if (MIXED && start[b]) {
        if (p < HW) {
            cur_disp[(size_t)b * HW + p] = 0.f;
            valid[(size_t)b * HW + p] = 0.f;
            flow[((size_t)b * 2 + 0) * HW + p] = 0.f;
            flow[((size_t)b * 2 + 1) * HW + p] = 0.f;
        }
        if (threadIdx.x == 0) partial[blockIdx.y * gridDim.x + blockIdx.x] = 0.f;
        return;
    }
    float cd = 0.f;
    if (p < HW) {
        const Cam c = load_cam(T_rel, K, K_inv, baseline, b);
        const int y = p / W, x = p - y * W;
        float zp, u, v;
        reproject(c, disp[(size_t)b * HW + p], (float)x, (float)y, zp, u, v);
        cd = fix_nonfinite(c.bf / zp);
        cur_disp[(size_t)b * HW + p] = cd;
        valid[(size_t)b * HW + p] = (cd > 0.f && cd < (float)W) ? 1.f : 0.f;
        flow[((size_t)b * 2 + 0) * HW + p] = u - (float)x;
        flow[((size_t)b * 2 + 1) * HW + p] = v - (float)y;
    }
    const float s = wave_sum(cd);
    if ((threadIdx.x & 63) == 0) red[threadIdx.x >> 6] = s;
    __syncthreads();
    if (threadIdx.x == 0) partial[blockIdx.y * gridDim.x + blockIdx.x] = (red[0] + red[1]) + (red[2] + red[3]);
}

__global__ __launch_bounds__(256) void k_warp_geometry(const float* __restrict__ disp, const float* __restrict__ T_rel,
                                                       const float* __restrict__ K, const float* __restrict__ K_inv,
                                                       const float* __restrict__ baseline, int H, int W,
                                                       float* __restrict__ cur_disp, float* __restrict__ valid,
                                                       float* __restrict__ flow, float* __restrict__ partial) {
    warp_geometry_body<false>(disp, T_rel, K, K_inv, baseline, nullptr, H, W, cur_disp, valid, flow, partial);
}

__global__ __launch_bounds__(256) void k_warp_geometry_mixed(const float* __restrict__ disp, const float* __restrict__ T_rel,
                                                             const float* __restrict__ K, const float* __restrict__ K_inv,
                                                             const float* __restrict__ baseline, const unsigned char* __restrict__ start,
                                                             int H, int W, float* __restrict__ cur_disp, float* __restrict__ valid,
                                                             float* __restrict__ flow, float* __restrict__ partial) {
    warp_geometry_body<true>(disp, T_rel, K, K_inv, baseline, start, H, W, cur_disp, valid, flow, partial);
}

__device__ __forceinline__ float partial_total(const float* __restrict__ partial, int n) {
    __shared__ float red[4];
    float s = 0.f;
    for (int i = threadIdx.x; i < n; i += 256) s += partial[i];
    s = wave_sum(s);
    if ((threadIdx.x & 63) == 0) red[threadIdx.x >> 6] = s;
    __syncthreads();
    return (red[0] + red[1]) + (red[2] + red[3]);
}

__global__ __launch_bounds__(256) void k_mean(const float* __restrict__ partial, int n, float inv_count, float* __restrict__ mean) {
    const float t = partial_total(partial, n);
    if (threadIdx.x == 0) *mean = t * inv_count;
}

__global__ __launch_bounds__(256) void k_mean_mixed(const float* __restrict__ partial, int n, const unsigned char* __restrict__ start, int B,
                                                    long long HW, float* __restrict__ mean) {
    const float t = partial_total(partial, n);
    if (threadIdx.x == 0) {
        long long count = 0;
        for (int b = 0; b < B; ++b) count += start[b] ? 0 : HW;
        *mean = count > 0 ? t * (1.0f / (float)count) : 0.f;
    }
}

__global__ __launch_bounds__(256) void k_metric(const float* __restrict__ cur_disp, const float* __restrict__ mean, int n,
                                                float* __restrict__ metric) {
    const int i = blockIdx.x * 256 + threadIdx.x;
    if (i < n) metric[i] = fminf(fmaxf(cur_disp[i] - *mean, -50.f), 50.f);
}

template <int MODE>
__global__ __launch_bounds__(256) void k_splat(const float* __restrict__ in, const float* __restrict__ flow,
                                               const float* __restrict__ cur_disp, const float* __restrict__ valid,
                                               const float* __restrict__ mean, int C, int H, int W, int ch_per_group,
                                               float* __restrict__ out) {
    const int b = blockIdx.y, HW = H * W;
    const int p = blockIdx.x * 256 + threadIdx.x;
    if (p >= HW) return;
    const int y = p / W, x = p - y * W;
    const float fx = (float)x + flow[((size_t)b * 2 + 0) * HW + p];
    const float fy = (float)y + flow[((size_t)b * 2 + 1) * HW + p];
    if (!isfinite(fx) || !isfinite(fy)) return;
    float scale = 1.f, cd = 0.f;
    if (MODE == 1) {
        if (valid[(size_t)b * HW + p] == 0.f) return;
        cd = cur_disp[(size_t)b * HW + p];
        scale = expf(fminf(fmaxf(cd - *mean, -50.f), 50.f));
    }
    const float x0f = floorf(fx), y0f = floorf(fy);
    if (!(x0f >= -2.f && x0f <= (float)W && y0f >= -2.f && y0f <= (float)H)) return;
    const int x0 = (int)x0f, y0 = (int)y0f;
    const float wnw = ((float)(x0 + 1) - fx) * ((float)(y0 + 1) - fy);
    const float wne = (fx - (float)x0) * ((float)(y0 + 1) - fy);
    const float wsw = ((float)(x0 + 1) - fx) * (fy - (float)y0);
    const float wse = (fx - (float)x0) * (fy - (float)y0);
    const bool xl = x0 >= 0 && x0 < W, xr = x0 + 1 >= 0 && x0 + 1 < W;
    const bool yt = y0 >= 0 && y0 < H, yb = y0 + 1 >= 0 && y0 + 1 < H;
    const int tnw = y0 * W + x0;
    const int Ctot = (MODE == 1) ? C + 2 : C;
    const int c_lo = blockIdx.z * ch_per_group, c_hi = min(Ctot, c_lo + ch_per_group);
    float* ob = out + (size_t)b * Ctot * HW;
    for (int c = c_lo; c < c_hi; ++c) {
        float v;
        if (MODE == 1) v = (c < C) ? in[((size_t)b * C + c) * HW + p] * scale : (c == C ? cd * scale : scale);
        else v = in[((size_t)b * C + c) * HW + p];
        float* o = ob + (size_t)c * HW + tnw;
        if (xl && yt) unsafeAtomicAdd(o, v * wnw);
        if (xr && yt) unsafeAtomicAdd(o + 1, v * wne);
        if (xl && yb) unsafeAtomicAdd(o + W, v * wsw);
        if (xr && yb) unsafeAtomicAdd(o + W + 1, v * wse);
    }
}

__global__ __launch_bounds__(256) void k_zero_fill(float4* __restrict__ p, size_t n4) {
    const size_t i = (size_t)blockIdx.x * 256 + threadIdx.x;
    if (i < n4) p[i] = make_float4(0.f, 0.f, 0.f, 0.f);
}

template <bool MIXED>
__device__ __forceinline__ bool finish_start(const unsigned char* __restrict__ start, const float* __restrict__ prior_disp,
                                             const float* __restrict__ prior_cost, const float* __restrict__ prior_mask, int C, int HW,
                                             float* __restrict__ out_disp, float* __restrict__ out_fmap, float* __restrict__ out_mask,
                                             float* __restrict__ out_cost) {
    const int b = blockIdx.y, lane = threadIdx.x & 63, q = threadIdx.x >> 6;
    if (!MIXED || !start[b]) return false;
    const int p = blockIdx.x * 64 + lane;
    if (p >= HW) return true;
    const size_t i = (size_t)b * HW + p;
    if (q == 0) {
        out_disp[i] = prior_disp[i];
        out_mask[i] = prior_mask[i];
        if (out_cost) out_cost[i] = prior_cost[i];
    }
    if (out_fmap) {
        const int cq = (C + 3) / 4, c_lo = q * cq, c_hi = min(C, c_lo + cq);
        for (int c = c_lo; c < c_hi; ++c) out_fmap[((size_t)b * C + c) * HW + p] = 0.f;
    }
    return true;
}

template <bool MIXED>
__device__ __forceinline__ void warp_finish_body(const float* __restrict__ acc, const float* __restrict__ cur_fmap,
                                                 const unsigned char* __restrict__ start, const float* __restrict__ prior_disp,
                                                 const float* __restrict__ prior_cost, const float* __restrict__ prior_mask,
                                                 int C, int HW, float* __restrict__ out_disp, float* __restrict__ out_fmap,
                                                 float* __restrict__ out_mask, float* __restrict__ out_cost) {
    __shared__ float s_part[3][4][64];
    if (finish_start<MIXED>(start, prior_disp, prior_cost, prior_mask, C, HW, out_disp, out_fmap, out_mask, out_cost)) return;
    const int b = blockIdx.y, lane = threadIdx.x & 63, q = threadIdx.x >> 6;
    const int p_raw = blockIdx.x * 64 + lane;
    const bool active = p_raw < HW;
    const int p = active ? p_raw : HW - 1;
    const float* a = acc + (size_t)b * (C + 2) * HW + p;
    const float norm = a[(size_t)(C + 1) * HW];
    const float mask = (norm != 0.f) ? 1.f : 0.f;
    const float den = fmaxf(norm, 1e-7f);
    if (q == 0 && active) {
        out_disp[(size_t)b * HW + p] = a[(size_t)C * HW] / den;
        out_mask[(size_t)b * HW + p] = mask;
    }
    const int cq = (C + 3) / 4, c_lo = q * cq, c_hi = min(C, c_lo + cq);
    float dot = 0.f, n1 = 0.f, nw = 0.f;
    for (int c = c_lo; c < c_hi; ++c) {
        const float fw = a[(size_t)c * HW] / den;
        if (out_fmap && active) out_fmap[((size_t)b * C + c) * HW + p] = fw;
        if (out_cost) {
            const float f1 = cur_fmap[((size_t)b * C + c) * HW + p];
            dot = fmaf(f1, fw, dot);
            n1 = fmaf(f1, f1, n1);
            nw = fmaf(fw, fw, nw);
        }
    }
    if (!out_cost) return;
    s_part[0][q][lane] = dot; s_part[1][q][lane] = n1; s_part[2][q][lane] = nw;
    __syncthreads();
    if (q == 0 && active) {
        float t[3];
#pragma unroll
        for (int k = 0; k < 3; ++k) t[k] = ((s_part[k][0][lane] + s_part[k][1][lane]) + s_part[k][2][lane]) + s_part[k][3][lane];
        out_cost[(size_t)b * HW + p] = t[0] / (fmaxf(sqrtf(t[1]), 1e-12f) * fmaxf(sqrtf(t[2]), 1e-12f)) * mask;
    }
}

__global__ __launch_bounds__(256) void k_warp_finish(const float* __restrict__ acc, const float* __restrict__ cur_fmap,
                                                     int C, int HW, float* __restrict__ out_disp, float* __restrict__ out_fmap,
                                                     float* __restrict__ out_mask, float* __restrict__ out_cost) {
    warp_finish_body<false>(acc, cur_fmap, nullptr, nullptr, nullptr, nullptr, C, HW, out_disp, out_fmap, out_mask, out_cost);
}

__global__ __launch_bounds__(256) void k_warp_finish_mixed(const float* __restrict__ acc, const float* __restrict__ cur_fmap,
                                                           const unsigned char* __restrict__ start, const float* __restrict__ prior_disp,
                                                           const float* __restrict__ prior_cost, const float* __restrict__ prior_mask,
                                                           int C, int HW, float* __restrict__ out_disp, float* __restrict__ out_fmap,
// ... 417 lines not shown
}

static bool ord_dims_ok(int B, int H, int W) { return (long long)B * 4 * H * W <= 0x7fffffffLL && B <= 65535; }

template <int MODE>
static void ord_index(const float* flow, const float* cur_disp, const float* valid, const float* mean, int B, int H, int W, const OrdWs& o,
                      hipStream_t s) {
    const int HW = H * W, nb = tcs_cdiv(HW, 256);
    const size_t n4 = o.count_bytes / 16;
    hipLaunchKernelGGL(k_zero_fill, dim3((unsigned)((n4 + 255) / 256)), dim3(256), 0, s, reinterpret_cast<float4*>(o.count), n4);
    hipLaunchKernelGGL(k_ord_count<MODE>, dim3(nb, B), dim3(256), 0, s, flow, cur_disp, valid, mean, H, W, o.count, o.scale);
    hipLaunchKernelGGL(k_ord_scan, dim3(B), dim3(1024), 0, s, o.count, HW, o.start, o.cursor, o.total);
    hipLaunchKernelGGL(k_ord_place<MODE>, dim3(nb, B), dim3(256), 0, s, flow, valid, H, W, o.cursor, o.slots);
    hipLaunchKernelGGL(k_ord_rank, dim3(tcs_cdiv(4LL * HW, 256), B), dim3(256), 0, s, o.slots, o.start, o.count, o.total, HW, o.sorted);
}

extern "C" {

size_t tcs_warp_ordered_workspace_bytes(int B, int C, int H, int W) {
    if (B <= 0 || C < 0 || H <= 0 || W <= 0) return 0;
    const size_t HW = (size_t)H * W;
    return al256(B * HW * 4) * 2 + al256(2 * B * HW * 4) + al256((size_t)B * tcs_cdiv(HW, 256) * 4) + 256 + ord_bytes(B, HW, true);
}

size_t tcs_softsplat_ordered_workspace_bytes(int B, int H, int W) {
    if (B <= 0 || H <= 0 || W <= 0) return 0;
    return ord_bytes(B, (size_t)H * W, false);
}

size_t tcs_warp_workspace_bytes(int B, int C, int H, int W) {
    if (B <= 0 || C < 0 || H <= 0 || W <= 0) return 0;
    const size_t HW = (size_t)H * W;
    return al256(B * HW * 4) * 2 + al256(2 * B * HW * 4) + al256((size_t)B * tcs_cdiv(HW, 256) * 4) + 256 +
           al256((size_t)B * (C + 2) * HW * 4);
}

static int geometry(const float* prev_disp, const float* T_rel, const float* K, const float* K_inv, const float* baseline,
                    int B, int H, int W, const WarpWs& w, hipStream_t s, const unsigned char* start = nullptr) {
    const int nb = tcs_cdiv((long long)H * W, 256);
    if (start) {
        hipLaunchKernelGGL(k_warp_geometry_mixed, dim3(nb, B), dim3(256), 0, s, prev_disp, T_rel, K, K_inv, baseline, start, H, W,
                           w.cur_disp, w.valid, w.flow, w.partial);
        hipLaunchKernelGGL(k_mean_mixed, dim3(1), dim3(256), 0, s, w.partial, nb * B, start, B, (long long)H * W, w.mean);
        return tcs_launch_status();
    }
    hipLaunchKernelGGL(k_warp_geometry, dim3(nb, B), dim3(256), 0, s, prev_disp, T_rel, K, K_inv, baseline, H, W,
                       w.cur_disp, w.valid, w.flow, w.partial);
    hipLaunchKernelGGL(k_mean, dim3(1), dim3(256), 0, s, w.partial, nb * B, 1.0f / (float)((long long)B * H * W), w.mean);
    return tcs_launch_status();
}

int tcs_warp_geometry(const float* prev_disp, const float* T_rel, const float* K, const float* K_inv,
                      const float* baseline, int B, int H, int W,
                      float* cur_disp, float* valid, float* flow, float* metric, void* workspace, tcs_stream_t stream) {
    if (!prev_disp || !T_rel || !K || !K_inv || !baseline || !cur_disp || !valid || !flow || !metric || !workspace)
        return TCS_EINVAL;
    if (B <= 0 || B > 65535 || H <= 0 || W <= 0) return TCS_EINVAL;
    hipStream_t s = tcs_stream(stream);
    WarpWs w = carve(workspace, B, 0, H, W);
    w.cur_disp = cur_disp; w.valid = valid; w.flow = flow;
    int rc = geometry(prev_disp, T_rel, K, K_inv, baseline, B, H, W, w, s);
    if (rc) return rc;
    const int n = B * H * W;
    hipLaunchKernelGGL(k_metric, dim3(tcs_cdiv(n, 256)), dim3(256), 0, s, cur_disp, w.mean, n, metric);
    return tcs_launch_status();
}

int tcs_warp_forward(const float* prev_disp, const float* prev_fmap, const float* T_rel, const float* K,
                     const float* K_inv, const float* baseline, int B, int C, int H, int W,
                     float* out_disp, float* out_fmap, float* out_mask, const float* cur_fmap, float* out_cost,
                     void* workspace, tcs_stream_t stream) {
    if (!prev_disp || !prev_fmap || !T_rel || !K || !K_inv || !baseline || !out_disp || !out_mask || !workspace)
        return TCS_EINVAL;
    if ((cur_fmap == nullptr) != (out_cost == nullptr)) return TCS_EINVAL;
    if (B <= 0 || B > 65535 || C <= 0 || H <= 0 || W <= 0) return TCS_EINVAL;
    hipStream_t s = tcs_stream(stream);
    WarpWs w = carve(workspace, B, C, H, W);
    int rc = geometry(prev_disp, T_rel, K, K_inv, baseline, B, H, W, w, s);
    if (rc) return rc;
    {
        const size_t n4 = (w.acc_bytes + 15) / 16;
        hipLaunchKernelGGL(k_zero_fill, dim3((unsigned)((n4 + 255) / 256)), dim3(256), 0, s, reinterpret_cast<float4*>(w.acc), n4);
    }
    const int nb = tcs_cdiv((long long)H * W, 256);
    const int cpg = 16, groups = tcs_cdiv(C + 2, cpg);
    hipLaunchKernelGGL(k_splat<1>, dim3(nb, B, groups), dim3(256), 0, s, prev_fmap, w.flow, w.cur_disp, w.valid, w.mean,
                       C, H, W, cpg, w.acc);
    hipLaunchKernelGGL(k_warp_finish, dim3(tcs_cdiv((long long)H * W, 64), B), dim3(256), 0, s, w.acc, cur_fmap, C, H * W, out_disp, out_fmap,
                       out_mask, out_cost);
    return tcs_launch_status();
}

int tcs_warp_forward_mixed(const float* prev_disp, const float* prev_fmap, const float* T_rel, const float* K,
                           const float* K_inv, const float* baseline, const unsigned char* start, const float* prior_disp,
                           const float* prior_cost, const float* prior_mask, int B, int C, int H, int W,
                           float* out_disp, float* out_fmap, float* out_mask, const float* cur_fmap, float* out_cost,
                           void* workspace, tcs_stream_t stream) {
    if (!prev_disp || !prev_fmap || !T_rel || !K || !K_inv || !baseline || !out_disp || !out_mask || !workspace)
        return TCS_EINVAL;
    if (!start || !prior_disp || !prior_cost || !prior_mask) return TCS_EINVAL;
    if ((cur_fmap == nullptr) != (out_cost == nullptr)) return TCS_EINVAL;
    if (B <= 0 || B > 65535 || C <= 0 || H <= 0 || W <= 0) return TCS_EINVAL;
    hipStream_t s = tcs_stream(stream);
    WarpWs w = carve(workspace, B, C, H, W);
    int rc = geometry(prev_disp, T_rel, K, K_inv, baseline, B, H, W, w, s, start);
    if (rc) return rc;
    {
        const size_t n4 = (w.acc_bytes + 15) / 16;
        hipLaunchKernelGGL(k_zero_fill, dim3((unsigned)((n4 + 255) / 256)), dim3(256), 0, s, reinterpret_cast<float4*>(w.acc), n4);
    }
    const int nb = tcs_cdiv((long long)H * W, 256);
    const int cpg = 16, groups = tcs_cdiv(C + 2, cpg);
    hipLaunchKernelGGL(k_splat<1>, dim3(nb, B, groups), dim3(256), 0, s, prev_fmap, w.flow, w.cur_disp, w.valid, w.mean,
                       C, H, W, cpg, w.acc);
    hipLaunchKernelGGL(k_warp_finish_mixed, dim3(tcs_cdiv((long long)H * W, 64), B), dim3(256), 0, s, w.acc, cur_fmap, start, prior_disp,
                       prior_cost, prior_mask, C, H * W, out_disp, out_fmap, out_mask, out_cost);
    return tcs_launch_status();
}

int tcs_softsplat_sum(const float* in, const float* flow, int B, int C, int H, int W, float* out, tcs_stream_t stream) {
    if (!in || !flow || !out || B <= 0 || B > 65535 || C <= 0 || H <= 0 || W <= 0) return TCS_EINVAL;
    const int nb = tcs_cdiv((long long)H * W, 256);
    const int cpg = 16, groups = tcs_cdiv(C, cpg);
    hipLaunchKernelGGL(k_splat<0>, dim3(nb, B, groups), dim3(256), 0, tcs_stream(stream), in, flow,
                       (const float*)nullptr, (const float*)nullptr, (const float*)nullptr, C, H, W, cpg, out);
    return tcs_launch_status();
}

int tcs_warp_forward_ordered(const float* prev_disp, const float* prev_fmap, const float* T_rel, const float* K,
                             const float* K_inv, const float* baseline, int B, int C, int H, int W,
                             float* out_disp, float* out_fmap, float* out_mask, const float* cur_fmap, float* out_cost,
                             void* workspace, tcs_stream_t stream) {
    if (!prev_disp || !prev_fmap || !T_rel || !K || !K_inv || !baseline || !out_disp || !out_mask || !workspace)
        return TCS_EINVAL;
    if ((cur_fmap == nullptr) != (out_cost == nullptr)) return TCS_EINVAL;
    if (B <= 0 || B > 65535 || C <= 0 || H <= 0 || W <= 0 || !ord_dims_ok(B, H, W)) return TCS_EINVAL;
    hipStream_t s = tcs_stream(stream);
    const WarpWs w = carve(workspace, B, C, H, W);
    int rc = geometry(prev_disp, T_rel, K, K_inv, baseline, B, H, W, w, s);
    if (rc) return rc;
    const OrdWs o = carve_ord(w.acc, B, (size_t)H * W, true);
    ord_index<1>(w.flow, w.cur_disp, w.valid, w.mean, B, H, W, o, s);
    hipLaunchKernelGGL(k_ord_warp_gather, dim3(tcs_cdiv((long long)H * W, 64), B), dim3(256), 0, s, o.start, o.count, o.sorted, prev_fmap,
                       w.cur_disp, o.scale, cur_fmap, C, H * W, out_disp, out_fmap, out_mask, out_cost);
    return tcs_launch_status();
}

int tcs_warp_forward_ordered_mixed(const float* prev_disp, const float* prev_fmap, const float* T_rel, const float* K,
                                   const float* K_inv, const float* baseline, const unsigned char* start, const float* prior_disp,
                                   const float* prior_cost, const float* prior_mask, int B, int C, int H, int W,
                                   float* out_disp, float* out_fmap, float* out_mask, const float* cur_fmap, float* out_cost,
                                   void* workspace, tcs_stream_t stream) {
    if (!prev_disp || !prev_fmap || !T_rel || !K || !K_inv || !baseline || !out_disp || !out_mask || !workspace)
        return TCS_EINVAL;
    if (!start || !prior_disp || !prior_cost || !prior_mask) return TCS_EINVAL;
    if ((cur_fmap == nullptr) != (out_cost == nullptr)) return TCS_EINVAL;
    if (B <= 0 || B > 65535 || C <= 0 || H <= 0 || W <= 0 || !ord_dims_ok(B, H, W)) return TCS_EINVAL;
    hipStream_t s = tcs_stream(stream);
    const WarpWs w = carve(workspace, B, C, H, W);
    int rc = geometry(prev_disp, T_rel, K, K_inv, baseline, B, H, W, w, s, start);
    if (rc) return rc;
    const OrdWs o = carve_ord(w.acc, B, (size_t)H * W, true);
    ord_index<1>(w.flow, w.cur_disp, w.valid, w.mean, B, H, W, o, s);
    hipLaunchKernelGGL(k_ord_warp_gather_mixed, dim3(tcs_cdiv((long long)H * W, 64), B), dim3(256), 0, s, o.start, o.count, o.sorted,
                       prev_fmap, w.cur_disp, o.scale, cur_fmap, start, prior_disp, prior_cost, prior_mask, C, H * W, out_disp, out_fmap,
                       out_mask, out_cost);
    return tcs_launch_status();
}

int tcs_softsplat_sum_ordered(const float* in, const float* flow, int B, int C, int H, int W, float* out, void* workspace,
                              tcs_stream_t stream) {
    if (!in || !flow || !out || !workspace || B <= 0 || B > 65535 || C <= 0 || H <= 0 || W <= 0 || !ord_dims_ok(B, H, W))
        return TCS_EINVAL;
    hipStream_t s = tcs_stream(stream);
    const OrdWs o = carve_ord(workspace, B, (size_t)H * W, false);
    ord_index<0>(flow, nullptr, nullptr, nullptr, B, H, W, o, s);
    hipLaunchKernelGGL(k_ord_sum_gather, dim3(tcs_cdiv((long long)H * W, 64), B), dim3(256), 0, s, o.start, o.count, o.sorted, in, C, H * W,
                       out);
    return tcs_launch_status();
}

int tcs_backward_grid(const float* disp, const float* T_rel, const float* K, const float* K_inv,
                      const float* baseline, int B, int H, int W, float* grid, tcs_stream_t stream) {
    if (!disp || !T_rel || !K || !K_inv || !baseline || !grid || B <= 0 || B > 65535 || H <= 0 || W <= 0) return TCS_EINVAL;
    hipLaunchKernelGGL(k_backward_grid, dim3(tcs_cdiv((long long)H * W, 256), B), dim3(256), 0, tcs_stream(stream),
                       disp, T_rel, K, K_inv, baseline, H, W, grid);
    return tcs_launch_status();
}

int tcs_bilinear_sample(const float* img, const float* grid, int B, int C, int Hi, int Wi, int Ho, int Wo,
                        float* out, tcs_stream_t stream) {
    if (!img || !grid || !out || B <= 0 || B > 65535 || C <= 0 || Hi <= 0 || Wi <= 0 || Ho <= 0 || Wo <= 0) return TCS_EINVAL;
    const int cpg = 16;
    hipLaunchKernelGGL(k_bilinear_sample, dim3(tcs_cdiv((long long)Ho * Wo, 256), B, tcs_cdiv(C, cpg)), dim3(256), 0,
                       tcs_stream(stream), img, grid, C, Hi, Wi, Ho * Wo, cpg, out);
    return tcs_launch_status();
}

int tcs_bilinear_sample_mixed(const float* img, const float* grid, const unsigned char* start, int B, int C, int Hi, int Wi, int Ho,
                              int Wo, float* out, tcs_stream_t stream) {
    if (!img || !grid || !start || !out || B <= 0 || B > 65535 || C <= 0 || Hi <= 0 || Wi <= 0 || Ho <= 0 || Wo <= 0) return TCS_EINVAL;
    const int cpg = 16;
    hipLaunchKernelGGL(k_bilinear_sample_mixed, dim3(tcs_cdiv((long long)Ho * Wo, 256), B, tcs_cdiv(C, cpg)), dim3(256), 0,
                       tcs_stream(stream), img, grid, start, C, Hi, Wi, Ho * Wo, cpg, out);
    return tcs_launch_status();
}

int tcs_grid_halve(const float* grid, int B, int H, int W, float* out, tcs_stream_t stream) {
// ... 43 lines not shown
```

### temporally-consistent-stereo-matching_amd/tcs_mi355/graph.py

```python
from __future__ import annotations

import gc
import warnings
from typing import Callable, Dict, List, Optional

import torch

_CAPTURING = 0


_OUTPUTS_KEYS = ("up", "q", "grad", "flow_mono", "flow_init", "cost_volume")


def _flatten(temporal):
    if temporal is None:
        return []
    K, T, Tp, base, last_disp, nets, fmap1 = temporal[:7]
    return [K, T, Tp, base, last_disp, *nets, fmap1, *temporal[7:]]


def _unflatten(flat):
    if not flat:
        return None
    if flat[-1].dtype == torch.uint8:
        return _unflatten(flat[:-1]) + (flat[-1],)
    return (flat[0], flat[1], flat[2], flat[3], flat[4], list(flat[5:-1]), flat[-1])


def _wants_argmax(temporal):
    return temporal is None or len(temporal) == 8


class _no_gc:

    def __enter__(self):
        global _CAPTURING
        self.was = gc.isenabled()
        gc.disable()
        _CAPTURING += 1

    def __exit__(self, *exc):
        global _CAPTURING
        _CAPTURING -= 1
        if self.was:
            gc.enable()
        return False


class _Slot:

    def __init__(self):
        self.feats = None
        self.token = None
        self.fresh = False
        self.by_prefetch = False
        self.age = 0
        self.ex_key = None


class _Entry:

    def __init__(self, graph, static_in, static_out, graph2=None, start=None):
        self.graph, self.static_in, self.static_out, self.graph2, self.start = graph, static_in, static_out, graph2, start


class FrameGraphs:

    def __init__(self, extract_fn: Callable, head_fn: Callable, loop_fn: Callable, warmup: int = 2,
                 epoch_fn: Optional[Callable[[], object]] = None, strict: bool = False):
        self.extract_fn, self.head_fn, self.loop_fn = extract_fn, head_fn, loop_fn
        self.warmup, self.epoch_fn, self.strict = warmup, epoch_fn, strict
        self.slots = [_Slot(), _Slot()]
        self.turn = 0
        self.ex: Dict[tuple, Optional[List[_Entry]]] = {}
        self.rf: Dict[tuple, Optional[List[_Entry]]] = {}
        self.epoch = epoch_fn() if epoch_fn is not None else None
        self.fell_back = 0
        self.captures = 0
        self.prefetched = 0

    @property
    def cache(self):
        return {**{("extract", *k): v for k, v in self.ex.items()}, **{("refine", *k): v for k, v in self.rf.items()}}

    def _check_epoch(self):
        if self.epoch_fn is not None:
            now = self.epoch_fn()
            if now != self.epoch:
                torch.cuda.synchronize()
# ... 85 lines not shown

    def prefetch(self, image1, image2, first: bool = False, use_graph: bool = True) -> int:
        self._check_epoch()
        token = self._token(image1, image2, first, use_graph)
        for k in (0, 1):
            if self.slots[k].fresh and self._same(self.slots[k].token, token):
                return k
        si = self._pick_slot()
        self._launch_extract(si, image1, image2, first, use_graph)
        self.slots[si].by_prefetch = True
        return si

    def _capture_refine(self, key, image1, image2, iters, flat, first, outputs=False) -> Optional[List[_Entry]]:
        ex_key = self._ex_key(image1, first, outputs)
        try:
            for si in (0, 1):
                if self.slots[si].feats is None or self.slots[si].ex_key != ex_key or self.ex.get(ex_key) is None \
                        or self.slots[si].feats is not self.ex[ex_key][si].static_out:
                    self._launch_extract(si, image1, image2, first, True, outputs=outputs)
            if self.ex.get(ex_key) is None:
                return None
            torch.cuda.synchronize()
            static_in = [t.detach().clone() if t.dtype == torch.uint8 else t.detach().float().clone() for t in flat]
            entries = []
            for si in (0, 1):
                feats = self.ex[ex_key][si].static_out
                run = lambda: self.loop_fn(feats, self.head_fn(feats, _unflatten(static_in)), iters, outputs)
                side = torch.cuda.Stream()
                side.wait_stream(torch.cuda.current_stream())
                with torch.cuda.stream(side):
                    for _ in range(self.warmup if si == 0 else 1):
                        run()
                torch.cuda.current_stream().wait_stream(side)
                torch.cuda.synchronize()
                g1, g2 = torch.cuda.CUDAGraph(), torch.cuda.CUDAGraph()
                with _no_gc(), torch.cuda.graph(g1):
                    start = self.head_fn(feats, _unflatten(static_in))
                g1.replay()
                with _no_gc(), torch.cuda.graph(g2):
                    out = self.loop_fn(feats, start, iters, outputs)
                g2.replay()
                entries.append(_Entry(g1, static_in, out, graph2=g2, start=start))
            torch.cuda.synchronize()
            self.captures += 1
            for sl in self.slots:
                sl.fresh, sl.token = False, None
            return entries
        except Exception as e:
            if self.strict:
                raise
            warnings.warn(f"HIP graph capture failed ({type(e).__name__}: {e}); running this shape with eager launches")
            torch.cuda.synchronize()
            return None

    def __call__(self, image1, image2, iters, temporal, use_graph: bool = True, outputs: bool = False):
        self._check_epoch()
        flat = _flatten(temporal)
        first = _wants_argmax(temporal)
        token = self._token(image1, image2, first, use_graph, outputs)
        entries = None
        if use_graph:
            key = self._rf_key(image1, iters, flat, outputs)
            if key not in self.rf:
                self.rf[key] = self._capture_refine(key, image1, image2, iters, flat, first, outputs)
            entries = self.rf[key]
            if entries is None:
                self.fell_back += 1
        si = next((k for k in (0, 1) if self.slots[k].fresh and self._same(self.slots[k].token, token)), None)
        for k in (0, 1):
            sl = self.slots[k]
            if sl.fresh and k != si:
                sl.age += 1
                if sl.age >= 2:
                    sl.fresh, sl.token = False, None
        if si is not None:
            self.prefetched += int(self.slots[si].by_prefetch)
        else:
            si = self._pick_slot()
            self._launch_extract(si, image1, image2, first, use_graph and entries is not None, outputs=outputs)
        slot = self.slots[si]
        slot.fresh, slot.token = False, None
        if entries is not None and self.ex.get(slot.ex_key) is not None and slot.feats is self.ex[slot.ex_key][si].static_out:
            e = entries[si]
            for dst, src in zip(e.static_in, flat):
                dst.copy_(src)
            e.graph.replay()
            e.graph2.replay()
            o = e.static_out
            out = {"flow": o["flow"].clone(), "flow_q": o["flow_q"].clone(), "net_list": [t.clone() for t in o["net_list"]],
                   "fmap1": o["fmap1"].clone()}
            for k in _OUTPUTS_KEYS if outputs else ():
                out[k] = o[k].clone()
        else:
            start = self.head_fn(slot.feats, temporal)
            if outputs:
                out = self.loop_fn(slot.feats, start, iters, True)
                out = dict(out, fmap1=out["fmap1"].clone(), cost_volume=out["cost_volume"].clone())
            else:
                out = self.loop_fn(slot.feats, start, iters)
                out = dict(out, fmap1=out["fmap1"].clone())
        return out
```

### temporally-consistent-stereo-matching_amd/tcs_mi355/native.py

```python
from __future__ import annotations

import ctypes as C
import os
import threading

import torch

from . import build as _build

_LIB = None
_LOCK = threading.Lock()

c_fp = C.c_void_p
c_int = C.c_int
c_f = C.c_float
c_sz = C.c_size_t


class ConvDesc(C.Structure):
    _fields_ = [
        ("src", c_fp * 4), ("src_ch", c_int * 4), ("n_src", c_int),
        ("weight", c_fp), ("bias", c_fp),
        ("B", c_int), ("H", c_int), ("W", c_int),
        ("Cin", c_int), ("Cout", c_int), ("ksize", c_int),
        ("epilogue", c_int), ("act", c_int), ("post_scale", c_f),
        ("addend", c_fp), ("addend2", c_fp), ("h", c_fp), ("z", c_fp),
        ("blend_keep_z", c_int),
        ("out", c_fp), ("out_ctot", c_int), ("out_coff", c_int), ("out2", c_fp),
        ("stride", c_int), ("math", c_int), ("weight_unscale", c_f),
        ("out16", c_fp), ("out16_groups", c_int), ("out16_group_offset", c_int),
        ("in_transform", c_int), ("src_batch2", c_fp), ("batch_split", c_int),
        ("products", c_int),
    ]


class ConvS16Desc(C.Structure):
    _fields_ = [
        ("src", c_fp * 4), ("src_ch", c_int * 4), ("src_groups", c_int * 4), ("n_src", c_int),
        ("weight", c_fp), ("bias", c_fp),
        ("B", c_int), ("H", c_int), ("W", c_int),
        ("Cin", c_int), ("Cout", c_int), ("ksize", c_int), ("stride", c_int),
        ("epilogue", c_int), ("act", c_int), ("post_scale", c_f), ("weight_unscale", c_f),
        ("addend", c_fp), ("addend2", c_fp), ("addend16", c_fp), ("addend16_groups", c_int), ("h", c_fp), ("h_groups", c_int), ("z", c_fp),
        ("blend_keep_z", c_int),
        ("out16", c_fp), ("out16_groups", c_int), ("out16_group_offset", c_int),
        ("out32", c_fp), ("out_ctot", c_int), ("out_coff", c_int),
        ("tile_cfg", c_int), ("addend_ctot", c_int),
        ("blend_cand", c_fp), ("blend_cand_ctot", c_int), ("blend_disp", c_fp), ("blend_refined", c_fp), ("blend_delta", c_fp),
        ("blend_coords1", c_fp), ("blend_flow_x", c_fp), ("blend_flow16", c_fp), ("blend_flow16_groups", c_int), ("blend_flow16_channel", c_int),
        ("out16b", c_fp), ("out16b_groups", c_int), ("out16_split", c_int),
        ("in_stats", c_fp), ("in_eps", c_f),
        ("tap_weights", c_fp), ("tap_out", c_fp), ("tap_nout", c_int), ("tap_tiles", c_int), ("tap_unscale", c_f),
        ("blend_warm_pyr", c_fp * 4), ("blend_warm_radius", c_int),
        ("products", c_int),
    ]


class S16Instance(C.Structure):
    _fields_ = [(n, c_int) for n in ("ksize", "stride", "epilogue", "mt", "rows", "ksteps", "nstage", "row_split", "rows_per_wave", "taps",
                                     "products", "csplit", "blocks", "threads")] + [("lds_bytes", C.c_longlong)]


SIGNATURES = {
    "tcs_abi_version": (c_int, []),
    "tcs_error_string": (C.c_char_p, [c_int]),
    "tcs_corr_level_bytes": (c_sz, [c_int, c_int, c_int, c_int]),
    "tcs_corr_build_workspace_bytes": (c_sz, [c_int, c_int, c_int]),
    "tcs_corr_build": (c_int, [c_fp, c_fp, c_int, c_int, c_int, c_int, c_fp, c_fp, c_fp, c_fp, c_fp, c_fp, c_fp, c_fp,
                               c_fp, c_fp, c_fp, c_fp, c_fp]),
    "tcs_corr_ws_level0": (c_fp, [c_fp]),
    "tcs_corr_lookup": (c_int, [c_fp, c_fp, c_fp, c_fp, c_fp, c_int, c_int, c_int, c_int, c_fp, c_fp, c_fp]),
    "tcs_corr_lookup_blocks": (c_int, [c_int, c_int, c_int]),
    "tcs_corr_lookup_backward": (c_int, [c_fp, c_fp, c_fp, c_fp, c_fp, c_fp, c_int, c_int, c_int, c_int, c_fp, c_fp, c_fp]),
    "tcs_corr_build_backward_scratch_bytes": (c_sz, [c_int, c_int, c_int, c_int]),
    "tcs_corr_build_backward": (c_int, [c_fp, c_fp, c_fp, c_fp, c_int, c_int, c_int, c_int, c_fp, c_fp, c_fp, c_fp]),
    "tcs_pose_prepare": (c_int, [c_fp, c_fp, c_fp, c_f, c_int, c_fp, c_fp, c_fp, c_fp, c_fp]),
    "tcs_pose_prepare_mixed": (c_int, [c_fp, c_fp, c_fp, c_fp, c_f, c_int, c_fp, c_fp, c_fp, c_fp, c_fp]),
    "tcs_warp_workspace_bytes": (c_sz, [c_int, c_int, c_int, c_int]),
    "tcs_warp_forward": (c_int, [c_fp, c_fp, c_fp, c_fp, c_fp, c_fp, c_int, c_int, c_int, c_int, c_fp, c_fp, c_fp, c_fp, c_fp,
                                 c_fp, c_fp]),
    "tcs_warp_geometry": (c_int, [c_fp, c_fp, c_fp, c_fp, c_fp, c_int, c_int, c_int, c_fp, c_fp, c_fp, c_fp, c_fp, c_fp]),
    "tcs_softsplat_sum": (c_int, [c_fp, c_fp, c_int, c_int, c_int, c_int, c_fp, c_fp]),
    "tcs_warp_ordered_workspace_bytes": (c_sz, [c_int, c_int, c_int, c_int]),
    "tcs_warp_forward_ordered": (c_int, [c_fp, c_fp, c_fp, c_fp, c_fp, c_fp, c_int, c_int, c_int, c_int, c_fp, c_fp, c_fp, c_fp, c_fp,
                                         c_fp, c_fp]),
    "tcs_warp_forward_mixed": (c_int, [c_fp, c_fp, c_fp, c_fp, c_fp, c_fp, c_fp, c_fp, c_fp, c_fp, c_int, c_int, c_int, c_int, c_fp,
                                       c_fp, c_fp, c_fp, c_fp, c_fp, c_fp]),
    "tcs_warp_forward_ordered_mixed": (c_int, [c_fp, c_fp, c_fp, c_fp, c_fp, c_fp, c_fp, c_fp, c_fp, c_fp, c_int, c_int, c_int, c_int,
                                               c_fp, c_fp, c_fp, c_fp, c_fp, c_fp, c_fp]),
    "tcs_softsplat_ordered_workspace_bytes": (c_sz, [c_int, c_int, c_int]),
    "tcs_softsplat_sum_ordered": (c_int, [c_fp, c_fp, c_int, c_int, c_int, c_int, c_fp, c_fp, c_fp]),
    "tcs_backward_grid": (c_int, [c_fp, c_fp, c_fp, c_fp, c_fp, c_int, c_int, c_int, c_fp, c_fp]),
    "tcs_bilinear_sample": (c_int, [c_fp, c_fp, c_int, c_int, c_int, c_int, c_int, c_int, c_fp, c_fp]),
    "tcs_bilinear_sample_mixed": (c_int, [c_fp, c_fp, c_fp, c_int, c_int, c_int, c_int, c_int, c_int, c_fp, c_fp]),
    "tcs_grid_halve": (c_int, [c_fp, c_int, c_int, c_int, c_fp, c_fp]),
    "tcs_flow_step": (c_int, [c_fp, c_fp, c_int, c_int, c_int, c_fp, c_fp]),
    "tcs_flow_step_grads": (c_int, [c_fp, c_fp, c_int, c_int, c_int, c_f, c_fp, c_fp, c_fp, c_fp]),
    "tcs_disp_gradient_xy": (c_int, [c_fp, c_int, c_int, c_int, c_f, c_fp, c_fp]),
    "tcs_grad_candidates": (c_int, [c_fp, c_int, c_int, c_int, c_fp, c_fp]),
    "tcs_propagate_disparity": (c_int, [c_fp, c_fp, c_int, c_int, c_int, c_fp, c_fp]),
    "tcs_softmax_blend": (c_int, [c_fp, c_fp, c_int, c_fp, c_int, c_int, c_int, c_fp, c_fp, c_fp, c_fp, c_fp, C.c_longlong, c_fp]),
    "tcs_convex_upsample": (c_int, [c_fp, c_fp, c_int, c_int, c_int, c_int, c_fp, c_fp, c_fp]),
    "tcs_convex_upsample_pair": (c_int, [c_fp, c_fp, c_fp, c_int, c_int, c_int, c_fp, c_fp, c_fp, c_fp, c_fp]),
    "tcs_avgpool3s2": (c_int, [c_fp, c_int, c_int, c_int, c_int, c_fp, c_fp]),
    "tcs_resize_bilinear": (c_int, [c_fp, c_int, c_int, c_int, c_int, c_int, c_int, c_fp, c_fp]),
    "tcs_resize_bilinear_scaled": (c_int, [c_fp, c_int, c_int, c_int, c_int, c_int, c_int, c_f, c_fp, c_fp]),
    "tcs_conv_packed_floats": (c_sz, [c_int, c_int, c_int]),
    "tcs_pack_conv_weight": (c_int, [c_fp, c_int, c_int, c_int, c_fp, c_fp]),
    "tcs_conv_packed_floats_f16x3": (c_sz, [c_int, c_int, c_int]),
    "tcs_pack_conv_weight_f16x3": (c_int, [c_fp, c_int, c_int, c_int, c_int, c_fp, c_fp]),
    "tcs_deconv_packed_floats_f16x3": (c_sz, [c_int, c_int]),
    "tcs_pack_deconv4x4s2_f16x3": (c_int, [c_fp, c_int, c_int, c_int, c_fp, c_fp, c_fp]),
    "tcs_instance_norm": (c_int, [c_fp, c_int, c_int, c_int, c_int, c_f, c_int, c_fp, c_fp, c_fp]),
    "tcs_conv3x3_cout1": (c_int, [c_fp, c_fp, c_fp, c_int, c_int, c_int, c_int, c_fp, c_fp]),
    "tcs_conv2d": (c_int, [C.POINTER(ConvDesc), c_fp]),
    "tcs_conv2d_group": (c_int, [C.POINTER(C.POINTER(ConvDesc)), c_int, c_fp]),
    "tcs_conv2d_group_fused": (c_int, [C.POINTER(C.POINTER(ConvDesc)), c_int]),
    "tcs_s16_bytes": (c_sz, [c_int, c_int, c_int, c_int]),
    "tcs_s16_flags": (c_int, [C.POINTER(C.c_uint)]),
    "tcs_s16_flags_detail": (c_int, [C.POINTER(C.c_uint)]),
    "tcs_s16_from_f32": (c_int, [c_fp, c_int, c_int, c_int, c_int, c_fp, c_int, c_int, c_fp]),
    "tcs_s16_to_f32": (c_int, [c_fp, c_int, c_int, c_int, c_int, c_int, c_int, c_fp, c_fp]),
    "tcs_conv2d_s16": (c_int, [C.POINTER(ConvS16Desc), c_fp]),
    "tcs_conv2d_s16_group": (c_int, [C.POINTER(C.POINTER(ConvS16Desc)), c_int, c_fp]),
    "tcs_conv2d_s16_group_fused": (c_int, [C.POINTER(C.POINTER(ConvS16Desc)), c_int]),
    "tcs_conv2d_s16_plan": (c_int, [C.POINTER(ConvS16Desc), C.POINTER(S16Instance)]),
    "tcs_avgpool3s2_s16": (c_int, [c_fp, c_int, c_int, c_int, c_int, c_fp, c_int, c_fp]),
    "tcs_resize_bilinear_s16": (c_int, [c_fp, c_int, c_int, c_int, c_int, c_int, c_int, c_fp, c_int, c_fp]),
    "tcs_instance_norm_s16_workspace_bytes": (c_sz, [c_int, c_int, c_int, c_int]),
    "tcs_instance_norm_s16": (c_int, [c_fp, c_int, c_int, c_int, c_int, c_f, c_int, c_fp, c_int, c_fp, c_int, c_fp, c_fp]),
    "tcs_deconv_in_stats_bytes": (c_sz, [c_int, c_int, c_int, c_int]),
    "tcs_instance_norm_apply_s16": (c_int, [c_fp, c_int, c_int, c_int, c_int, c_int, c_fp, c_int, c_fp, c_int, c_fp, c_int, c_f, c_fp]),
    "tcs_tap_weights_floats": (c_sz, [c_int, c_int]),
    "tcs_pack_tap_weights": (c_int, [c_fp, c_int, c_int, c_int, c_fp, c_fp]),
    "tcs_taps_sum": (c_int, [c_fp, c_int, c_int, c_fp, c_fp, c_f, c_int, c_int, c_int, c_fp, c_fp]),
    "tcs_flow_taps_step_grads": (c_int, [c_fp, c_fp, c_int, c_fp, c_int, c_int, c_int, c_f, c_fp, c_fp, c_fp, c_fp, c_fp]),
    "tcs_taps_propagate_s16": (c_int, [c_fp, c_int, c_fp, c_fp, c_f, c_fp, c_int, c_int, c_int, c_fp, c_fp, c_fp, c_int, c_fp]),
    "tcs_propagate_disparity_s16": (c_int, [c_fp, c_fp, c_int, c_int, c_int, c_fp, c_fp, c_int, c_fp]),
    "tcs_s16_set_channel": (c_int, [c_fp, c_int, c_int, c_int, c_fp, c_int, c_int, c_fp]),
    "tcs_weight_frags_bytes": (c_sz, [c_int, c_int]),
    "tcs_pack_weight_frags": (c_int, [c_fp, c_int, c_int, c_int, c_int, c_fp, c_fp]),
    "tcs_hidden_update_s16": (c_int, [c_fp, c_int, c_fp, c_fp, c_fp, c_fp, c_fp, c_f, c_fp, c_fp, c_f, c_fp, c_fp, c_f, c_int, c_int, c_int, c_fp]),
    "tcs_softmax_blend_s16": (c_int, [c_fp, c_fp, c_int, c_fp, c_int, c_int, c_int, c_fp, c_fp, c_fp, c_fp, c_fp, c_int, c_int, c_fp]),
    "tcs_loss_workspace_bytes": (c_sz, [c_int, c_int, c_int, c_int]),
    "tcs_loss_targets": (c_int, [c_fp, c_fp, c_int, c_int, c_int, c_int, c_fp, c_fp, c_fp, c_fp, c_fp, c_fp, c_fp]),
    "tcs_loss_targets_full": (c_int, [c_fp, c_int, c_fp, c_int, c_int, c_int, c_int, c_fp, c_fp, c_fp, c_fp, c_fp]),
    "tcs_sequence_loss": (c_int, [c_fp, C.c_longlong, C.c_longlong, c_int, c_fp, c_fp, c_int, c_fp, c_fp, c_int, c_int, c_int, c_fp,
                                  c_fp]),
    "tcs_init_loss": (c_int, [c_fp, c_int, c_fp, c_fp, c_int, c_int, c_int, c_int, c_int, c_f, c_int, c_fp, c_fp]),
    "tcs_grad_normal_loss": (c_int, [c_fp, C.c_longlong, c_fp, C.c_longlong, C.c_longlong, c_int, c_fp, c_fp, c_fp, c_fp, c_fp, c_fp,
                                     c_int, c_int, c_int, c_fp, c_fp]),
    "tcs_loss_finish": (c_int, [c_fp, c_int, c_int, c_int, c_int, c_int, c_int, C.POINTER(C.c_double), c_fp, c_fp, c_fp]),
    "tcs_loss_finish_counts": (c_int, [c_fp, c_int, c_int, c_int, c_int, c_int, c_int, C.POINTER(C.c_double), c_fp, c_fp, c_fp, c_fp]),
    "tcs_sequence_loss_bwd": (c_int, [c_fp, C.c_longlong, C.c_longlong, c_int, c_fp, c_fp, c_int, c_fp, c_fp, c_int, c_int, c_int,
                                      C.POINTER(C.c_double), c_fp, c_fp, c_fp, c_fp, c_fp, c_fp]),
    "tcs_init_loss_bwd": (c_int, [c_fp, c_int, c_fp, c_fp, c_int, c_int, c_int, c_int, c_int, c_f, c_fp, c_fp, c_fp, c_fp]),
    "tcs_grad_normal_loss_bwd": (c_int, [c_fp, C.c_longlong, c_fp, C.c_longlong, C.c_longlong, c_int, c_fp, c_fp, c_fp, c_fp, c_fp, c_fp,
                                         c_int, c_int, c_int, C.POINTER(C.c_double), c_fp, c_fp, c_fp, c_fp, c_fp]),
    "tcs_upsample_flow": (c_int, [c_fp, c_fp, c_int, c_int, c_int, c_fp, c_fp]),
    "tcs_upsample_flow_pair": (c_int, [c_fp, c_fp, c_fp, c_int, c_int, c_int, c_fp, c_fp, c_fp]),
    "tcs_convex_upsample_backward_workspace_floats": (c_sz, [c_int, c_int, c_int, c_int]),
    "tcs_convex_upsample_backward": (c_int, [c_fp, c_fp, c_fp, c_int, c_int, c_int, c_fp, c_fp, c_fp, c_fp]),
    "tcs_convex_upsample_pair_backward": (c_int, [c_fp, c_fp, c_fp, c_fp, c_int, c_int, c_int, c_fp, c_fp, c_fp, c_fp, c_fp]),
    "tcs_refine_blend": (c_int, [c_fp, c_fp, c_fp, c_int, c_int, c_int, c_fp, c_fp]),
    "tcs_refine_blend_backward": (c_int, [c_fp, c_fp, c_fp, c_fp, c_int, c_int, c_int, c_fp, c_fp, c_fp]),
}


class NativeLibraryMissing(RuntimeError):
    pass


def lib_path() -> str:
    return os.environ.get("TCS_MI355_LIB", _build.LIB_PATH)


def lib():
    global _LIB
    if _LIB is None:
        with _LOCK:
            if _LIB is None:
                path = lib_path()
                if not os.path.exists(path):
                    raise NativeLibraryMissing(
                        f"{path} not found. The TC-Stereo hot path has no CPU or PyTorch fallback: build the HIP "
                        f"library first (python -c 'import __graft_entry__ as g; g.build()').")
                handle = C.CDLL(path)
                for name, (res, args) in SIGNATURES.items():
                    fn = getattr(handle, name)
                    fn.restype = res
                    fn.argtypes = args
                _LIB = handle
    return _LIB


def check(rc: int, what: str):
    if rc != 0:
        msg = lib().tcs_error_string(rc).decode()
        raise RuntimeError(f"{what} failed: {msg} ({rc})")


def ptr(t: torch.Tensor | None, name: str = "tensor", dtype=torch.float32):
    if t is None:
        return None
# ... 13 lines not shown
```

### temporally-consistent-stereo-matching_amd/tcs_mi355/ops.py

```python
from __future__ import annotations

import ctypes as C
from dataclasses import dataclass
from typing import List, Optional, Sequence

import torch

from . import grouping as _grouping
from . import native as nv

ACT = {"none": 0, "relu": 1, "sigmoid": 2, "tanh": 3, "leaky": 4, "relu_add_relu": 5}
EPI_LINEAR, EPI_GRU_ZR, EPI_GRU_Q = 0, 1, 2


def _new(like: torch.Tensor, *shape) -> torch.Tensor:
    return torch.empty(shape, dtype=torch.float32, device=like.device)


def _dims4(t: torch.Tensor, name: str):
    if t.ndim != 4:
        raise ValueError(f"{name}: expected a 4-D NCHW tensor, got shape {tuple(t.shape)}")
    return tuple(int(s) for s in t.shape)


@dataclass
class CorrPyramid:
    levels: List[torch.Tensor]
    B: int
    H: int
    W: int
    workspace: torch.Tensor
    natural: Optional[List[torch.Tensor]] = None
    cost_volume: Optional[torch.Tensor] = None
    sparse: Optional[tuple] = None


def corr_build(fmap1: torch.Tensor, fmap2: torch.Tensor, argmax: bool = False, cost_volume: bool = False,
               natural: bool = False) -> CorrPyramid:
    B, Cc, H, W = _dims4(fmap1, "fmap1")
    if tuple(fmap2.shape) != (B, Cc, H, W):
        raise ValueError(f"fmap2 shape {tuple(fmap2.shape)} != fmap1 shape {tuple(fmap1.shape)}")
    L = nv.lib()
    ws_bytes = L.tcs_corr_build_workspace_bytes(B, H, W)
    ws = torch.empty(ws_bytes // 4, dtype=torch.float32, device=fmap1.device)
    levels = [_new(fmap1, B, H, W >> i, W) for i in range(4)]
    nat = [None] * 4
    if natural:
        nat = [None] + [_new(fmap1, B, H, W, W >> i) for i in range(1, 4)]
    cost = _new(fmap1, B, W, H, W) if cost_volume else None
    sp = tuple(_new(fmap1, B, 1, H, W) for _ in range(3)) if argmax else (None, None, None)
    rc = L.tcs_corr_build(nv.ptr(fmap1, "fmap1"), nv.ptr(fmap2, "fmap2"), B, Cc, H, W,
                          *[nv.ptr(t) for t in levels], nv.ptr(nat[1]), nv.ptr(nat[2]), nv.ptr(nat[3]), nv.ptr(cost),
                          nv.ptr(sp[0]), nv.ptr(sp[1]), nv.ptr(sp[2]), nv.ptr(ws), nv.stream())
    nv.check(rc, "tcs_corr_build")
    out = CorrPyramid(levels, B, H, W, ws, cost_volume=cost, sparse=sp if argmax else None)
    if natural:
        out.natural = [ws[: B * H * W * W].view(B, H, W, W)] + nat[1:]
    return out


def corr_lookup(pyr: CorrPyramid, coords: torch.Tensor, radius: int = 4, out: Optional[torch.Tensor] = None) -> torch.Tensor:
    if tuple(coords.shape) != (pyr.B, 1, pyr.H, pyr.W):
        raise ValueError(f"coords shape {tuple(coords.shape)} != {(pyr.B, 1, pyr.H, pyr.W)}")
    n_ch = 4 * (2 * radius + 1)
    if out is None:
        out = _new(coords, pyr.B, n_ch, pyr.H, pyr.W)
    elif tuple(out.shape) != (pyr.B, n_ch, pyr.H, pyr.W):
        raise ValueError("corr_lookup: bad `out` shape")
    stamps = LOOKUP_PROBE.next_slot(pyr) if LOOKUP_PROBE is not None else None
    rc = nv.lib().tcs_corr_lookup(*[nv.ptr(t) for t in pyr.levels], nv.ptr(coords, "coords"), pyr.B, pyr.H, pyr.W, radius,
                                  nv.ptr(out, "out"), stamps, nv.stream())
    nv.check(rc, "tcs_corr_lookup")
    return out


def corr_lookup_backward(pyr: CorrPyramid, coords: torch.Tensor, grad_out: torch.Tensor, radius: int = 4,
                         want_vol: bool = True, want_coords: bool = False):
    B, H, W = pyr.B, pyr.H, pyr.W
    if tuple(coords.shape) != (B, 1, H, W):
        raise ValueError(f"coords shape {tuple(coords.shape)} != {(B, 1, H, W)}")
    n_ch = 4 * (2 * radius + 1)
    if tuple(grad_out.shape) != (B, n_ch, H, W):
        raise ValueError(f"grad_out shape {tuple(grad_out.shape)} != {(B, n_ch, H, W)}")
    gv = _new(coords, B, H, W, W) if want_vol else None
    gc = _new(coords, B, 1, H, W) if want_coords else None
    rc = nv.lib().tcs_corr_lookup_backward(*[nv.ptr(t) for t in pyr.levels], nv.ptr(coords, "coords"),
                                           nv.ptr(grad_out, "grad_out"), B, H, W, radius, nv.ptr(gv, "grad_vol"),
                                           nv.ptr(gc, "grad_coords"), nv.stream())
    nv.check(rc, "tcs_corr_lookup_backward")
    return gv, gc


def corr_build_backward(fmap1: torch.Tensor, fmap2: torch.Tensor, pyr: CorrPyramid, grad_vol: torch.Tensor,
                        want1: bool = True, want2: bool = True):
    B, Cc, H, W = _dims4(fmap1, "fmap1")
    if tuple(fmap2.shape) != (B, Cc, H, W):
        raise ValueError(f"fmap2 shape {tuple(fmap2.shape)} != fmap1 shape {tuple(fmap1.shape)}")
    if (pyr.B, pyr.H, pyr.W) != (B, H, W):
        raise ValueError("corr_build_backward: the pyramid was built from maps of another shape")
    if tuple(grad_vol.shape) != (B, H, W, W):
        raise ValueError(f"grad_vol shape {tuple(grad_vol.shape)} != {(B, H, W, W)}")
    L = nv.lib()
    g1 = _new(fmap1, B, Cc, H, W) if want1 else None
    g2 = _new(fmap1, B, Cc, H, W) if want2 else None
    sb = L.tcs_corr_build_backward_scratch_bytes(B, Cc, H, W)
# ... 725 lines not shown
```

### temporally-consistent-stereo-matching_amd/tcs_mi355/s16.py

```python
from __future__ import annotations

import ctypes as C
from dataclasses import dataclass
from typing import Dict, Optional, Sequence

import torch

from . import grouping as _grouping
from . import native as nv
from .ops import ACT, EPI_GRU_Q, EPI_GRU_ZR, EPI_LINEAR, MATH_F16X3, PackedConv

EPI_DECONV2X = 3
EPI_BLEND9 = 4


def groups_for(C_: int) -> int:
    return (C_ + 15) // 16 * 2


_CONV_GROUPS = _grouping.Family("s16", nv.ConvS16Desc, "tcs_conv2d_s16", "tcs_conv2d_s16_group", "tcs_conv2d_s16_group_fused")


class grouped(_grouping.Grouped):
    family = _CONV_GROUPS


_launch = _CONV_GROUPS.launch


@dataclass
class S16:
    data: torch.Tensor
    C: int

    @property
    def B(self):
        return int(self.data.shape[0])

    @property
    def G(self):
        return int(self.data.shape[1])

    @property
    def H(self):
        return int(self.data.shape[3]) - 2

    @property
    def W(self):
        return int(self.data.shape[4]) - 2

    @property
    def device(self):
        return self.data.device

    def ptr(self):
        return nv.ptr(self.data, "s16", dtype=torch.float16)

    def float(self) -> torch.Tensor:
        return from_s16(self)


def zeros(B: int, C_: int, H: int, W: int, device, groups: Optional[int] = None) -> S16:
    G = groups_for(C_) if groups is None else int(groups)
    return S16(torch.zeros(B, G, 2, H + 2, W + 2, 8, dtype=torch.float16, device=device), C_)


class S16Pool:

    def __init__(self, products: int = 0):
        self.buffers: Dict[tuple, S16] = {}
        self.products = int(products)

    def get(self, key, B, C_, H, W, device, groups=None) -> S16:
        G = groups_for(C_) if groups is None else int(groups)
        k = (key, B, C_, H, W, G, str(device))
        buf = self.buffers.get(k)
        if buf is None:
            buf = zeros(B, C_, H, W, device, G)
            self.buffers[k] = buf
        return buf

    def get32(self, key, shape, device, zero: bool = False) -> torch.Tensor:
        k = (key, tuple(int(v) for v in shape), "f32", str(device))
        buf = self.buffers.get(k)
        if buf is None:
            buf = self.buffers[k] = (torch.zeros if zero else torch.empty)(*k[1], dtype=torch.float32, device=device)
        return buf

    def get_i64(self, key, shape, device) -> torch.Tensor:
        k = (key, tuple(int(v) for v in shape), "i64", str(device))
        buf = self.buffers.get(k)
        if buf is None:
            buf = self.buffers[k] = torch.zeros(*k[1], dtype=torch.int64, device=device)
        return buf

    def bytes(self) -> int:
        return sum((b.data if isinstance(b, S16) else b).numel() * (b.data if isinstance(b, S16) else b).element_size() for b in self.buffers.values())


def to_s16(x: torch.Tensor, out: Optional[S16] = None, group_offset: int = 0) -> S16:
    if x.ndim != 4:
        raise ValueError("to_s16 expects [B,C,H,W]")
    B, C_, H, W = (int(v) for v in x.shape)
    if out is None:
        out = zeros(B, C_, H, W, x.device)
    elif (out.B, out.H, out.W) != (B, H, W):
        raise ValueError("to_s16: `out` has another shape")
    nv.check(nv.lib().tcs_s16_from_f32(nv.ptr(x, "x"), B, C_, H, W, out.ptr(), out.G, int(group_offset), nv.stream()), "tcs_s16_from_f32")
    return out


def from_s16(s: S16, C_: Optional[int] = None, group_offset: int = 0, out: Optional[torch.Tensor] = None) -> torch.Tensor:
    C_ = s.C if C_ is None else int(C_)
    if out is None:
        out = torch.empty(s.B, C_, s.H, s.W, dtype=torch.float32, device=s.device)
    nv.check(nv.lib().tcs_s16_to_f32(s.ptr(), s.B, C_, s.H, s.W, s.G, int(group_offset), nv.ptr(out, "out"), nv.stream()), "tcs_s16_to_f32")
    return out


def _desc(pc: PackedConv, srcs: Sequence[S16], stride: int = 1) -> nv.ConvS16Desc:
    if pc.math != MATH_F16X3:
        raise ValueError("S16 convolutions need fp16-split packed weights (pack_conv(..., 'f16x3'))")
    if not 1 <= len(srcs) <= 4:
        raise ValueError("1..4 sources")
    d = nv.ConvS16Desc()
    B, H, W = srcs[0].B, srcs[0].H, srcs[0].W
    tot = 0
    for i, s in enumerate(srcs):
        if (s.B, s.H, s.W) != (B, H, W):
            raise ValueError(f"src{i} grid {(s.B, s.H, s.W)} does not match src0 {(B, H, W)}")
        d.src[i], d.src_ch[i], d.src_groups[i] = s.ptr(), s.C, s.G
        tot += s.C
    if tot != pc.cin:
        raise ValueError(f"sources carry {tot} channels, convolution expects {pc.cin}")
    d.n_src = len(srcs)
    d.weight, d.bias = nv.ptr(pc.weight), nv.ptr(pc.bias)
    d.B, d.H, d.W, d.Cin, d.Cout, d.ksize, d.stride = B, H, W, pc.cin, pc.cout, pc.ksize, stride
    d.post_scale, d.weight_unscale = 1.0, pc.unscale
    d.products = pc.products
    return d


def _slice_ptr(t: Optional[torch.Tensor], ctot: int, c: int, grid, name: str):
    if t is None:
        return None
    B, H, W = grid
    if not ctot:
        return nv.ptr(t, name)
    if t.dtype != torch.float32 or tuple(t.shape) != (B, c, H, W) or t.stride() != (ctot * H * W, H * W, W, 1):
        raise ValueError(f"{name}: expected a channel slice of a contiguous fp32 [B,{ctot},H,W] tensor")
    if not t.is_cuda:
        raise RuntimeError(f"{name}: tcs_mi355 kernels need a HIP device tensor")
    return t.data_ptr()


def _out_grid(s: S16, stride: int):
    return ((s.H - 1) // 2 + 1, (s.W - 1) // 2 + 1) if stride == 2 else (s.H, s.W)


def conv2d(pc: PackedConv, srcs: Sequence[S16], act: str = "none", addend: Optional[torch.Tensor] = None, post_scale: float = 1.0,
           out16: Optional[S16] = None, out16_group_offset: int = 0, out32: Optional[torch.Tensor] = None, out_coff: int = 0,
           stride: int = 1, want32: bool = False, tile_cfg: int = 0, addend16: Optional[S16] = None, addend_ctot: int = 0,
           out16b: Optional[S16] = None, out16_split: int = 0, taps: Optional["Taps"] = None, tap_weights: Optional["FragWeights"] = None):
    d = _desc(pc, srcs, stride)
    Ho, Wo = _out_grid(srcs[0], stride)
    if out32 is None and want32:
        out32 = torch.empty(d.B, pc.cout, Ho, Wo, dtype=torch.float32, device=srcs[0].device)
    if out16 is None and out32 is None and taps is None:
        out16 = zeros(d.B, pc.cout, Ho, Wo, srcs[0].device)
    if out16 is not None and (out16.B, out16.H, out16.W) != (d.B, Ho, Wo):
        raise ValueError("conv2d: bad `out16` grid")
    if out32 is not None and (out32.shape[0] != d.B or tuple(out32.shape[2:]) != (Ho, Wo)):
        raise ValueError("conv2d: bad `out32` shape")
    if addend is not None and not addend_ctot and tuple(addend.shape) != (d.B, pc.cout, Ho, Wo):
        raise ValueError("conv2d: bad addend shape")
    d.epilogue, d.act, d.post_scale = EPI_LINEAR, ACT[act], float(post_scale)
    d.addend, d.addend_ctot = _slice_ptr(addend, addend_ctot, pc.cout, (d.B, Ho, Wo), "addend"), int(addend_ctot)
    if addend16 is not None:
        if (addend16.B, addend16.H, addend16.W) != (d.B, Ho, Wo):
            raise ValueError("conv2d: bad addend16 grid")
        d.addend16, d.addend16_groups = addend16.ptr(), addend16.G
    if out16 is not None:
        d.out16, d.out16_groups, d.out16_group_offset = out16.ptr(), out16.G, int(out16_group_offset)
    if out16b is not None:
        if (out16 is None and taps is None) or (out16b.B, out16b.H, out16b.W) != (d.B, Ho, Wo):
            raise ValueError("conv2d: `out16b` needs `out16` (or `taps`) and the same grid")
        d.out16b, d.out16b_groups, d.out16_split = out16b.ptr(), out16b.G, int(out16_split)
    if taps is not None:
        if tap_weights is None or tuple(taps.data.shape) != (d.B, taps.ntile, 9 * taps.nout, Ho, Wo):
            raise ValueError("conv2d: `taps` needs `tap_weights` and a [B, ntile, 9*nout, H, W] buffer")
        if tap_weights.data.numel() < nv.lib().tcs_tap_weights_floats(taps.nout, 32 * taps.ntile):
            raise ValueError("conv2d: `tap_weights` too small")
# ... 270 lines not shown
```

Measured before the change: 37.81.

## Batch f32-to-s16 conversions and tensor copies into single launches; restructure splat kernel

Adds a multi-tensor f32-to-s16 conversion kernel and a multi-buffer copy kernel. Per-tensor conversion loops, the graph-replay input copies and the output clones now go through these, cutting kernel launch counts. Separately, the softsplat kernel is rewritten: one wavefront computes bilinear weights and masks for 64 pixels into shared memory, each block handles 32 channels, and adjacent-pixel contributions are merged via shuffles to reduce atomics. Costs are extra code complexity, and the single-pass splat may change the order of atomic accumulation.

```diff
diff --git a/include/tcs_mi355.h b/include/tcs_mi355.h
--- a/include/tcs_mi355.h
+++ b/include/tcs_mi355.h
@@ -191,6 +191,14 @@
 #define TCS_S16_FLAG_UNITS 5
 int tcs_s16_flags_detail(unsigned int* per_unit);
 int tcs_s16_from_f32(const float* x, int B, int C, int H, int W, void* s16, int groups_total, int group_offset, tcs_stream_t stream);
+#define TCS_S16_FROM_F32_MANY 4
+typedef struct tcs_s16_from_f32_desc {
+    const float* x;
+    int B, C, H, W;
+    void* s16;
+    int groups_total, group_offset;
+} tcs_s16_from_f32_desc;
+int tcs_s16_from_f32_many(const tcs_s16_from_f32_desc* descs, int n, tcs_stream_t stream);
 int tcs_s16_to_f32(const void* s16, int B, int C, int H, int W, int groups_total, int group_offset, float* out, tcs_stream_t stream);
 
 typedef struct tcs_conv_s16_desc {
@@ -346,6 +354,14 @@
 int tcs_refine_blend_backward(const float* logits9, const float* disp_grads, const float* disp, const float* grad_refined, int B, int H,
                               int W, float* grad_logits, float* grad_disp_grads, tcs_stream_t stream);
 
+#define TCS_COPY_MANY 16
+typedef struct tcs_copy_entry {
+    const void* src;
+    void* dst;
+    size_t bytes;
+} tcs_copy_entry;
+int tcs_copy_many(const tcs_copy_entry* entries, int n, tcs_stream_t stream);
+
 #ifdef __cplusplus
 }
 #endif
diff --git a/temporally-consistent-stereo-matching_amd/core/tc_stereo.py b/temporally-consistent-stereo-matching_amd/core/tc_stereo.py
--- a/temporally-consistent-stereo-matching_amd/core/tc_stereo.py
+++ b/temporally-consistent-stereo-matching_amd/core/tc_stereo.py
@@ -250,11 +250,11 @@
                 if i + 1 < len(last_net_list):
                     grid = ops.grid_halve(grid)
 
-        for i, (h, fuse) in enumerate(zip(net_list, self.previous_current_hideen_fuse)):
-            if warped is None:
-                x = pool.get(("frame", "zero", i), h.B, h.C, h.H, h.W, h.device)
-            else:
-                x = s16.to_s16(warped[i], out=pool.get(("frame", "warped", i), h.B, h.C, h.H, h.W, h.device))
+        if warped is None:
+            xs = [pool.get(("frame", "zero", i), h.B, h.C, h.H, h.W, h.device) for i, h in enumerate(net_list)]
+        else:
+            xs = s16.to_s16_many(warped, [pool.get(("frame", "warped", i), h.B, h.C, h.H, h.W, h.device) for i, h in enumerate(net_list)])
+        for h, x, fuse in zip(net_list, xs, self.previous_current_hideen_fuse):
             fuse.step16(pool, h, [x])
 
         coords0 = self._coords0(fmap1)
@@ -275,8 +275,9 @@
 
         pool = self._s16pool
         n3 = a.n_gru_layers == 3
-        grads16 = [s16.to_s16(t.float().contiguous(), out=pool.get(("frame", "ctxg", i), t.shape[0], t.shape[1], t.shape[2], t.shape[3], t.device))
-                   for i, t in enumerate(grad_list)]
+        grads16 = s16.to_s16_many([t.float().contiguous() for t in grad_list],
+                                  [pool.get(("frame", "ctxg", i), t.shape[0], t.shape[1], t.shape[2], t.shape[3], t.device)
+                                   for i, t in enumerate(grad_list)])
         dg_pre = self.disp_grad_refine.prepare(pool, grads16)
         self.disp_grad_refine.begin_frame(pool, coords1.shape[0], coords1.device)
         refined = up_mask = None
diff --git a/temporally-consistent-stereo-matching_amd/core/update.py b/temporally-consistent-stereo-matching_amd/core/update.py
--- a/temporally-consistent-stereo-matching_amd/core/update.py
+++ b/temporally-consistent-stereo-matching_amd/core/update.py
@@ -127,6 +127,11 @@
 def to16(pool, x, key):
     B, C_, H, W = (int(v) for v in x.shape)
     return s16.to_s16(x.float().contiguous(), out=pool.get(key, B, C_, H, W, x.device))
+
+
+def to16_many(pool, xs, keys):
+    xs = [x.float().contiguous() for x in xs]
+    return s16.to_s16_many(xs, [pool.get(key, *(int(v) for v in x.shape), x.device) for x, key in zip(xs, keys)])
 
 
 IN_SUM_SLOTS = 64
@@ -598,7 +603,7 @@
             y = conv16(pool, seq[0], srcs)
             return conv16(pool, seq[3], [s16.instance_norm(y, act="relu", out=y)], act=act)
 
-        c16 = [to16(pool, c, (id(self), "ctx", i)) for i, c in enumerate(ctx)]
+        c16 = to16_many(pool, ctx, [(id(self), "ctx", i) for i in range(len(ctx))])
         x4_disp = conv16(pool, self.conv_disp_fuse[2], [conv16(pool, self.conv_disp_fuse[0], [stem(self.conv_disp_stem, d),
                          stem(self.conv_cost_stem, cost), stem(self.conv_mask_stem, mask - 0.5)], act="relu")])
         x4 = cin(self.conv_4_4, [x4_disp, c16[0]])
diff --git a/temporally-consistent-stereo-matching_amd/csrc/tcs_conv_s16.hip b/temporally-consistent-stereo-matching_amd/csrc/tcs_conv_s16.hip
--- a/temporally-consistent-stereo-matching_amd/csrc/tcs_conv_s16.hip
+++ b/temporally-consistent-stereo-matching_amd/csrc/tcs_conv_s16.hip
@@ -557,12 +557,10 @@
     }
 }
 
-__global__ __launch_bounds__(256) void k_s16_from_f32(const float* __restrict__ x, int C, int H, int W, int G, int goff, int Gtot,
-                                                       _Float16* __restrict__ out) {
+__device__ __forceinline__ void s16_from_f32_unit(const float* __restrict__ x, int C, int H, int W, int G, int goff, int Gtot,
+                                                  _Float16* __restrict__ out, int b, size_t i) {
     const int HW = H * W;
     const size_t n = (size_t)G * HW;
-    const size_t i = (size_t)blockIdx.x * 256 + threadIdx.x;
-    const int b = blockIdx.y;
     if (i >= n) return;
     const int g = (int)(i / HW), p = (int)(i - (size_t)g * HW);
     const int y = p / W, xx = p - y * W;
@@ -581,6 +579,32 @@
     _Float16* o = out + s16_unit(b, Gtot, goff + g, 0, H + 2, W + 2, y, xx);
     *reinterpret_cast<half8*>(o) = hi;
     *reinterpret_cast<half8*>(o + (size_t)(H + 2) * (W + 2) * 8) = lo;
+}
+
+__global__ __launch_bounds__(256) void k_s16_from_f32(const float* __restrict__ x, int C, int H, int W, int G, int goff, int Gtot,
+                                                       _Float16* __restrict__ out) {
+    s16_from_f32_unit(x, C, H, W, G, goff, Gtot, out, blockIdx.y, (size_t)blockIdx.x * 256 + threadIdx.x);
+}
+
+struct FromF32ManyArgs {
+    const float* x[TCS_S16_FROM_F32_MANY];
+    _Float16* out[TCS_S16_FROM_F32_MANY];
+    int C[TCS_S16_FROM_F32_MANY], H[TCS_S16_FROM_F32_MANY], W[TCS_S16_FROM_F32_MANY], G[TCS_S16_FROM_F32_MANY];
+    int goff[TCS_S16_FROM_F32_MANY], Gtot[TCS_S16_FROM_F32_MANY];
+    unsigned per[TCS_S16_FROM_F32_MANY], first[TCS_S16_FROM_F32_MANY];
+};
+
+__global__ __launch_bounds__(256) void k_s16_from_f32_many(FromF32ManyArgs a) {
+    const unsigned bid = blockIdx.x;
+    int k = 0;
+#pragma unroll
+    for (int j = 1; j < TCS_S16_FROM_F32_MANY; ++j) k = bid >= a.first[j] ? j : k;
+#pragma unroll
+    for (int j = 0; j < TCS_S16_FROM_F32_MANY; ++j) {
+        if (j != k) continue;
+        const unsigned r = bid - a.first[j], b = r / a.per[j], blk = r - b * a.per[j];
+        s16_from_f32_unit(a.x[j], a.C[j], a.H[j], a.W[j], a.G[j], a.goff[j], a.Gtot[j], a.out[j], (int)b, (size_t)blk * 256 + threadIdx.x);
+    }
 }
 
 __global__ __launch_bounds__(256) void k_s16_to_f32(const _Float16* __restrict__ s, int C, int H, int W, int Gtot, int goff,
@@ -800,6 +824,32 @@
     const size_t n = (size_t)G * H * W;
     hipLaunchKernelGGL(k_s16_from_f32, dim3((unsigned)((n + 255) / 256), B), dim3(256), 0, tcs_stream(stream), x, C, H, W, G, group_offset,
                        groups_total, reinterpret_cast<_Float16*>(s16));
+    return tcs_launch_status();
+}
+
+int tcs_s16_from_f32_many(const tcs_s16_from_f32_desc* descs, int n, tcs_stream_t stream) {
+    if (n < 0 || n > TCS_S16_FROM_F32_MANY || !descs) return TCS_EINVAL;
+    if (n == 0) return TCS_OK;
+    FromF32ManyArgs a;
+    unsigned long long blocks = 0;
+    for (int k = 0; k < TCS_S16_FROM_F32_MANY; ++k) {
+        if (k >= n) {
+            a.x[k] = nullptr; a.out[k] = nullptr; a.C[k] = a.H[k] = a.W[k] = a.G[k] = a.goff[k] = a.Gtot[k] = 0;
+            a.per[k] = 1; a.first[k] = 0xffffffffu;
+            continue;
+        }
+        const tcs_s16_from_f32_desc& d = descs[k];
+        if (!d.x || !d.s16 || d.B <= 0 || d.B > 65535 || d.C <= 0 || d.H <= 0 || d.W <= 0) return TCS_EINVAL;
+        const int G = ((d.C + 15) / 16) * 2;
+        if (d.group_offset < 0 || (d.group_offset & 1) || d.group_offset + G > d.groups_total) return TCS_EINVAL;
+        const unsigned long long per = ((unsigned long long)G * d.H * d.W + 255) / 256;
+        a.x[k] = d.x; a.out[k] = reinterpret_cast<_Float16*>(d.s16);
+        a.C[k] = d.C; a.H[k] = d.H; a.W[k] = d.W; a.G[k] = G; a.goff[k] = d.group_offset; a.Gtot[k] = d.groups_total;
+        a.per[k] = (unsigned)per; a.first[k] = (unsigned)blocks;
+        blocks += per * d.B;
+        if (per > 0x7fffffffULL || blocks > 0x7fffffffULL) return TCS_EUNSUPPORTED;
+    }
+    hipLaunchKernelGGL(k_s16_from_f32_many, dim3((unsigned)blocks), dim3(256), 0, tcs_stream(stream), a);
     return tcs_launch_status();
 }
 
diff --git a/temporally-consistent-stereo-matching_amd/csrc/tcs_stencil.hip b/temporally-consistent-stereo-matching_amd/csrc/tcs_stencil.hip
--- a/temporally-consistent-stereo-matching_amd/csrc/tcs_stencil.hip
+++ b/temporally-consistent-stereo-matching_amd/csrc/tcs_stencil.hip
@@ -572,6 +572,55 @@
     dgrad[((size_t)b * 2 + 1) * HW + y * W + x] = ay;
 }
 
+#define CM_CHUNK 16384
+struct CopyManyArgs {
+    const char* src[TCS_COPY_MANY];
+    char* dst[TCS_COPY_MANY];
+    unsigned long long bytes[TCS_COPY_MANY];
+    unsigned first[TCS_COPY_MANY];
+};
+
+__global__ __launch_bounds__(256) void k_copy_many(CopyManyArgs a) {
+    const unsigned bid = blockIdx.x;
+    const char* s = a.src[0];
+    char* d = a.dst[0];
+    unsigned long long total = a.bytes[0];
+    unsigned f = 0;
+#pragma unroll
+    for (int k = 1; k < TCS_COPY_MANY; ++k) {
+        const bool here = bid >= a.first[k];
+        s = here ? a.src[k] : s;
+        d = here ? a.dst[k] : d;
+        total = here ? a.bytes[k] : total;
+        f = here ? a.first[k] : f;
+    }
+    const unsigned long long off = (unsigned long long)(bid - f) * CM_CHUNK;
+    const unsigned len = (unsigned)(total - off < (unsigned long long)CM_CHUNK ? total - off : (unsigned long long)CM_CHUNK);
+    s += off;
+    d += off;
+    const unsigned long long both = (unsigned long long)(uintptr_t)s | (unsigned long long)(uintptr_t)d;
+    unsigned done = 0;
+    if ((both & 15) == 0) {
+        const unsigned n16 = len >> 4;
+        const uint4* s4 = reinterpret_cast<const uint4*>(s);
+        uint4* d4 = reinterpret_cast<uint4*>(d);
+        if (n16 == CM_CHUNK / 16) {
+            const uint4 v0 = s4[threadIdx.x], v1 = s4[threadIdx.x + 256], v2 = s4[threadIdx.x + 512], v3 = s4[threadIdx.x + 768];
+            d4[threadIdx.x] = v0; d4[threadIdx.x + 256] = v1; d4[threadIdx.x + 512] = v2; d4[threadIdx.x + 768] = v3;
+        } else {
+            for (unsigned i = threadIdx.x; i < n16; i += 256) d4[i] = s4[i];
+        }
+        done = n16 << 4;
+    } else if ((both & 3) == 0) {
+        const unsigned n4 = len >> 2;
+        const unsigned* s1 = reinterpret_cast<const unsigned*>(s);
+        unsigned* d1 = reinterpret_cast<unsigned*>(d);
+        for (unsigned i = threadIdx.x; i < n4; i += 256) d1[i] = s1[i];
+        done = n4 << 2;
+    }
+    for (unsigned i = done + threadIdx.x; i < len; i += 256) d[i] = s[i];
+}
+
 extern "C" {
 
 size_t tcs_tap_weights_floats(int nout, int C) {
@@ -753,7 +802,7 @@
     return tcs_launch_status();
 }
 
-int tcs_abi_version(void) { return 17; }
+int tcs_abi_version(void) { return 18; }
 
 const char* tcs_error_string(int code) {
     switch (code) {
@@ -765,6 +814,28 @@
     }
 }
 
+int tcs_copy_many(const tcs_copy_entry* entries, int n, tcs_stream_t stream) {
+    if (n < 0 || n > TCS_COPY_MANY || !entries) return TCS_EINVAL;
+    CopyManyArgs a;
+    unsigned long long blocks = 0;
+    int m = 0;
+    for (int i = 0; i < n; ++i) {
+        if (entries[i].bytes == 0) continue;
+        if (!entries[i].src || !entries[i].dst) return TCS_EINVAL;
+        a.src[m] = reinterpret_cast<const char*>(entries[i].src);
+        a.dst[m] = reinterpret_cast<char*>(entries[i].dst);
+        a.bytes[m] = entries[i].bytes;
+        a.first[m] = (unsigned)blocks;
+        blocks += (entries[i].bytes + CM_CHUNK - 1) / CM_CHUNK;
+        if (blocks > 0x7fffffffULL) return TCS_EUNSUPPORTED;
+        ++m;
+    }
+    if (m == 0) return TCS_OK;
+    for (int k = m; k < TCS_COPY_MANY; ++k) { a.src[k] = nullptr; a.dst[k] = nullptr; a.bytes[k] = 0; a.first[k] = 0xffffffffu; }
+    hipLaunchKernelGGL(k_copy_many, dim3((unsigned)blocks), dim3(256), 0, tcs_stream(stream), a);
+    return tcs_launch_status();
+}
+
 }
 
 int tcs_s16_flag_take_stencil(unsigned int* out) {
diff --git a/temporally-consistent-stereo-matching_amd/csrc/tcs_warp.hip b/temporally-consistent-stereo-matching_amd/csrc/tcs_warp.hip
--- a/temporally-consistent-stereo-matching_amd/csrc/tcs_warp.hip
+++ b/temporally-consistent-stereo-matching_amd/csrc/tcs_warp.hip
@@ -115,46 +115,73 @@
     if (i < n) metric[i] = fminf(fmaxf(cur_disp[i] - *mean, -50.f), 50.f);
 }
 
+#define SPLAT_CH 32
 template <int MODE>
 __global__ __launch_bounds__(256) void k_splat(const float* __restrict__ in, const float* __restrict__ flow,
                                                const float* __restrict__ cur_disp, const float* __restrict__ valid,
-                                               const float* __restrict__ mean, int C, int H, int W, int ch_per_group,
-                                               float* __restrict__ out) {
+                                               const float* __restrict__ mean, int C, int H, int W, float* __restrict__ out) {
+    __shared__ float s_w[4][64], s_scale[64], s_cd[64];
+    __shared__ int s_tnw[64], s_mask[64];
     const int b = blockIdx.y, HW = H * W;
-    const int p = blockIdx.x * 256 + threadIdx.x;
-    if (p >= HW) return;
-    const int y = p / W, x = p - y * W;
-    const float fx = (float)x + flow[((size_t)b * 2 + 0) * HW + p];
-    const float fy = (float)y + flow[((size_t)b * 2 + 1) * HW + p];
-    if (!isfinite(fx) || !isfinite(fy)) return;
-    float scale = 1.f, cd = 0.f;
-    if (MODE == 1) {
-        if (valid[(size_t)b * HW + p] == 0.f) return;
-        cd = cur_disp[(size_t)b * HW + p];
-        scale = expf(fminf(fmaxf(cd - *mean, -50.f), 50.f));
-    }
-    const float x0f = floorf(fx), y0f = floorf(fy);
-    if (!(x0f >= -2.f && x0f <= (float)W && y0f >= -2.f && y0f <= (float)H)) return;
-    const int x0 = (int)x0f, y0 = (int)y0f;
-    const float wnw = ((float)(x0 + 1) - fx) * ((float)(y0 + 1) - fy);
-    const float wne = (fx - (float)x0) * ((float)(y0 + 1) - fy);
-    const float wsw = ((float)(x0 + 1) - fx) * (fy - (float)y0);
-    const float wse = (fx - (float)x0) * (fy - (float)y0);
-    const bool xl = x0 >= 0 && x0 < W, xr = x0 + 1 >= 0 && x0 + 1 < W;
-    const bool yt = y0 >= 0 && y0 < H, yb = y0 + 1 >= 0 && y0 + 1 < H;
-    const int tnw = y0 * W + x0;
+    const int lane = threadIdx.x & 63, wv = threadIdx.x >> 6;
+    const int p = blockIdx.x * 64 + lane;
+    if (wv == 0) {
+        int m = 0, tnw = 0;
+        float w[4] = {0.f, 0.f, 0.f, 0.f}, scale = 1.f, cd = 0.f;
+        if (p < HW) {
+            const int y = p / W, x = p - y * W;
+            const float fx = (float)x + flow[((size_t)b * 2 + 0) * HW + p];
+            const float fy = (float)y + flow[((size_t)b * 2 + 1) * HW + p];
+            bool ok = isfinite(fx) && isfinite(fy);
+            if (MODE == 1) ok = ok && valid[(size_t)b * HW + p] != 0.f;
+            const float x0f = floorf(fx), y0f = floorf(fy);
+            ok = ok && (x0f >= -2.f && x0f <= (float)W && y0f >= -2.f && y0f <= (float)H);
+            if (ok) {
+                if (MODE == 1) {
+                    cd = cur_disp[(size_t)b * HW + p];
+                    scale = expf(fminf(fmaxf(cd - *mean, -50.f), 50.f));
+                }
+                const int x0 = (int)x0f, y0 = (int)y0f;
+                w[0] = ((float)(x0 + 1) - fx) * ((float)(y0 + 1) - fy);
+                w[1] = (fx - (float)x0) * ((float)(y0 + 1) - fy);
+                w[2] = ((float)(x0 + 1) - fx) * (fy - (float)y0);
+                w[3] = (fx - (float)x0) * (fy - (float)y0);
+                const bool xl = x0 >= 0 && x0 < W, xr = x0 + 1 >= 0 && x0 + 1 < W;
+                const bool yt = y0 >= 0 && y0 < H, yb = y0 + 1 >= 0 && y0 + 1 < H;
+                tnw = y0 * W + x0;
+                m = (xl && yt ? 1 : 0) | (xr && yt ? 2 : 0) | (xl && yb ? 4 : 0) | (xr && yb ? 8 : 0);
+            }
+        }
+        const int m_next = __shfl_down(m, 1, 64), t_next = __shfl_down(tnw, 1, 64);
+        const bool adj = lane < 63 && t_next == tnw + 1;
+        const int give = ((adj && (m & 2) && (m_next & 1)) ? 16 : 0) | ((adj && (m & 8) && (m_next & 4)) ? 32 : 0);
+        const int give_prev = __shfl_up(give, 1, 64);
+        m |= give | (lane > 0 ? (give_prev << 2) : 0);
+        s_tnw[lane] = tnw; s_mask[lane] = m; s_scale[lane] = scale; s_cd[lane] = cd;
+#pragma unroll
+        for (int k = 0; k < 4; ++k) s_w[k][lane] = w[k];
+    }
+    __syncthreads();
+    const int m = s_mask[lane], tnw = s_tnw[lane];
+    const float wnw = s_w[0][lane], wne = s_w[1][lane], wsw = s_w[2][lane], wse = s_w[3][lane];
+    const float scale = s_scale[lane], cd = s_cd[lane];
+    const bool live = (m & 15) != 0;
     const int Ctot = (MODE == 1) ? C + 2 : C;
-    const int c_lo = blockIdx.z * ch_per_group, c_hi = min(Ctot, c_lo + ch_per_group);
+    const int c_lo = blockIdx.z * SPLAT_CH, c_hi = min(Ctot, c_lo + SPLAT_CH);
     float* ob = out + (size_t)b * Ctot * HW;
-    for (int c = c_lo; c < c_hi; ++c) {
-        float v;
-        if (MODE == 1) v = (c < C) ? in[((size_t)b * C + c) * HW + p] * scale : (c == C ? cd * scale : scale);
-        else v = in[((size_t)b * C + c) * HW + p];
+    for (int c = c_lo + wv; c < c_hi; c += 4) {
+        float v = 0.f;
+        if (live) {
+            if (MODE == 1) v = (c < C) ? in[((size_t)b * C + c) * HW + p] * scale : (c == C ? cd * scale : scale);
+            else v = in[((size_t)b * C + c) * HW + p];
+        }
+        const float ne = v * wne, se = v * wse;
+        const float ne_prev = __shfl_up(ne, 1, 64), se_prev = __shfl_up(se, 1, 64);
         float* o = ob + (size_t)c * HW + tnw;
-        if (xl && yt) unsafeAtomicAdd(o, v * wnw);
-        if (xr && yt) unsafeAtomicAdd(o + 1, v * wne);
-        if (xl && yb) unsafeAtomicAdd(o + W, v * wsw);
-        if (xr && yb) unsafeAtomicAdd(o + W + 1, v * wse);
+        if (m & 1) unsafeAtomicAdd(o, (m & 64) ? v * wnw + ne_prev : v * wnw);
+        if ((m & 2) && !(m & 16)) unsafeAtomicAdd(o + 1, ne);
+        if (m & 4) unsafeAtomicAdd(o + W, (m & 128) ? v * wsw + se_prev : v * wsw);
+        if ((m & 8) && !(m & 32)) unsafeAtomicAdd(o + W + 1, se);
     }
 }
 
@@ -738,10 +765,8 @@
         const size_t n4 = (w.acc_bytes + 15) / 16;
         hipLaunchKernelGGL(k_zero_fill, dim3((unsigned)((n4 + 255) / 256)), dim3(256), 0, s, reinterpret_cast<float4*>(w.acc), n4);
     }
-    const int nb = tcs_cdiv((long long)H * W, 256);
-    const int cpg = 16, groups = tcs_cdiv(C + 2, cpg);
-    hipLaunchKernelGGL(k_splat<1>, dim3(nb, B, groups), dim3(256), 0, s, prev_fmap, w.flow, w.cur_disp, w.valid, w.mean,
-                       C, H, W, cpg, w.acc);
+    hipLaunchKernelGGL(k_splat<1>, dim3(tcs_cdiv((long long)H * W, 64), B, tcs_cdiv(C + 2, SPLAT_CH)), dim3(256), 0, s, prev_fmap, w.flow,
+                       w.cur_disp, w.valid, w.mean, C, H, W, w.acc);
     hipLaunchKernelGGL(k_warp_finish, dim3(tcs_cdiv((long long)H * W, 64), B), dim3(256), 0, s, w.acc, cur_fmap, C, H * W, out_disp, out_fmap,
                        out_mask, out_cost);
     return tcs_launch_status();
@@ -765,10 +790,8 @@
         const size_t n4 = (w.acc_bytes + 15) / 16;
         hipLaunchKernelGGL(k_zero_fill, dim3((unsigned)((n4 + 255) / 256)), dim3(256), 0, s, reinterpret_cast<float4*>(w.acc), n4);
     }
-    const int nb = tcs_cdiv((long long)H * W, 256);
-    const int cpg = 16, groups = tcs_cdiv(C + 2, cpg);
-    hipLaunchKernelGGL(k_splat<1>, dim3(nb, B, groups), dim3(256), 0, s, prev_fmap, w.flow, w.cur_disp, w.valid, w.mean,
-                       C, H, W, cpg, w.acc);
+    hipLaunchKernelGGL(k_splat<1>, dim3(tcs_cdiv((long long)H * W, 64), B, tcs_cdiv(C + 2, SPLAT_CH)), dim3(256), 0, s, prev_fmap, w.flow,
+                       w.cur_disp, w.valid, w.mean, C, H, W, w.acc);
     hipLaunchKernelGGL(k_warp_finish_mixed, dim3(tcs_cdiv((long long)H * W, 64), B), dim3(256), 0, s, w.acc, cur_fmap, start, prior_disp,
                        prior_cost, prior_mask, C, H * W, out_disp, out_fmap, out_mask, out_cost);
     return tcs_launch_status();
@@ -776,10 +799,9 @@
 
 int tcs_softsplat_sum(const float* in, const float* flow, int B, int C, int H, int W, float* out, tcs_stream_t stream) {
     if (!in || !flow || !out || B <= 0 || B > 65535 || C <= 0 || H <= 0 || W <= 0) return TCS_EINVAL;
-    const int nb = tcs_cdiv((long long)H * W, 256);
-    const int cpg = 16, groups = tcs_cdiv(C, cpg);
-    hipLaunchKernelGGL(k_splat<0>, dim3(nb, B, groups), dim3(256), 0, tcs_stream(stream), in, flow,
-                       (const float*)nullptr, (const float*)nullptr, (const float*)nullptr, C, H, W, cpg, out);
+    if (tcs_cdiv(C, SPLAT_CH) > 65535) return TCS_EUNSUPPORTED;
+    hipLaunchKernelGGL(k_splat<0>, dim3(tcs_cdiv((long long)H * W, 64), B, tcs_cdiv(C, SPLAT_CH)), dim3(256), 0, tcs_stream(stream), in, flow,
+                       (const float*)nullptr, (const float*)nullptr, (const float*)nullptr, C, H, W, out);
     return tcs_launch_status();
 }
 
diff --git a/temporally-consistent-stereo-matching_amd/tcs_mi355/graph.py b/temporally-consistent-stereo-matching_amd/tcs_mi355/graph.py
--- a/temporally-consistent-stereo-matching_amd/tcs_mi355/graph.py
+++ b/temporally-consistent-stereo-matching_amd/tcs_mi355/graph.py
@@ -5,6 +5,8 @@
 from typing import Callable, Dict, List, Optional
 
 import torch
+
+from . import ops
 
 _CAPTURING = 0
 
@@ -256,15 +258,14 @@
         slot.fresh, slot.token = False, None
         if entries is not None and self.ex.get(slot.ex_key) is not None and slot.feats is self.ex[slot.ex_key][si].static_out:
             e = entries[si]
-            for dst, src in zip(e.static_in, flat):
-                dst.copy_(src)
+            ops.copy_many(list(zip(e.static_in, flat)))
             e.graph.replay()
             e.graph2.replay()
             o = e.static_out
-            out = {"flow": o["flow"].clone(), "flow_q": o["flow_q"].clone(), "net_list": [t.clone() for t in o["net_list"]],
-                   "fmap1": o["fmap1"].clone()}
-            for k in _OUTPUTS_KEYS if outputs else ():
-                out[k] = o[k].clone()
+            keys = ["flow", "flow_q", "fmap1"] + (list(_OUTPUTS_KEYS) if outputs else [])
+            nets = len(o["net_list"])
+            fresh = ops.clone_many(list(o["net_list"]) + [o[k] for k in keys])
+            out = dict(zip(keys, fresh[nets:]), net_list=fresh[:nets])
         else:
             start = self.head_fn(slot.feats, temporal)
             if outputs:
diff --git a/temporally-consistent-stereo-matching_amd/tcs_mi355/native.py b/temporally-consistent-stereo-matching_amd/tcs_mi355/native.py
--- a/temporally-consistent-stereo-matching_amd/tcs_mi355/native.py
+++ b/temporally-consistent-stereo-matching_amd/tcs_mi355/native.py
@@ -54,6 +54,19 @@
         ("blend_warm_pyr", c_fp * 4), ("blend_warm_radius", c_int),
         ("products", c_int),
     ]
+
+
+class CopyEntry(C.Structure):
+    _fields_ = [("src", c_fp), ("dst", c_fp), ("bytes", c_sz)]
+
+
+class S16FromF32Desc(C.Structure):
+    _fields_ = [("x", c_fp), ("B", c_int), ("C", c_int), ("H", c_int), ("W", c_int), ("s16", c_fp), ("groups_total", c_int),
+                ("group_offset", c_int)]
+
+
+COPY_MANY = 16
+S16_FROM_F32_MANY = 4
 
 
 class S16Instance(C.Structure):
@@ -120,6 +133,8 @@
     "tcs_s16_flags": (c_int, [C.POINTER(C.c_uint)]),
     "tcs_s16_flags_detail": (c_int, [C.POINTER(C.c_uint)]),
     "tcs_s16_from_f32": (c_int, [c_fp, c_int, c_int, c_int, c_int, c_fp, c_int, c_int, c_fp]),
+    "tcs_s16_from_f32_many": (c_int, [C.POINTER(S16FromF32Desc), c_int, c_fp]),
+    "tcs_copy_many": (c_int, [C.POINTER(CopyEntry), c_int, c_fp]),
     "tcs_s16_to_f32": (c_int, [c_fp, c_int, c_int, c_int, c_int, c_int, c_int, c_fp, c_fp]),
     "tcs_conv2d_s16": (c_int, [C.POINTER(ConvS16Desc), c_fp]),
     "tcs_conv2d_s16_group": (c_int, [C.POINTER(C.POINTER(ConvS16Desc)), c_int, c_fp]),
diff --git a/temporally-consistent-stereo-matching_amd/tcs_mi355/ops.py b/temporally-consistent-stereo-matching_amd/tcs_mi355/ops.py
--- a/temporally-consistent-stereo-matching_amd/tcs_mi355/ops.py
+++ b/temporally-consistent-stereo-matching_amd/tcs_mi355/ops.py
@@ -21,6 +21,33 @@
     if t.ndim != 4:
         raise ValueError(f"{name}: expected a 4-D NCHW tensor, got shape {tuple(t.shape)}")
     return tuple(int(s) for s in t.shape)
+
+
+def _plain_copy(dst: torch.Tensor, src: torch.Tensor) -> bool:
+    return (isinstance(src, torch.Tensor) and dst.is_cuda and src.is_cuda and dst.device == src.device and dst.dtype == src.dtype
+            and dst.shape == src.shape and dst.is_contiguous() and src.is_contiguous())
+
+
+def copy_many(pairs: Sequence[tuple]) -> None:
+    plain = []
+    for dst, src in pairs:
+        if _plain_copy(dst, src):
+            if dst.numel() and dst.data_ptr() != src.data_ptr():
+                plain.append((dst, src))
+        else:
+            dst.copy_(src)
+    L = nv.lib()
+    for i in range(0, len(plain), nv.COPY_MANY):
+        part = plain[i:i + nv.COPY_MANY]
+        table = (nv.CopyEntry * len(part))(*[nv.CopyEntry(src.data_ptr(), dst.data_ptr(), dst.numel() * dst.element_size())
+                                              for dst, src in part])
+        nv.check(L.tcs_copy_many(table, len(part), nv.stream()), "tcs_copy_many")
+
+
+def clone_many(tensors: Sequence[torch.Tensor]) -> List[torch.Tensor]:
+    out = [torch.empty_like(t) if (t.is_cuda and t.is_contiguous()) else t.clone() for t in tensors]
+    copy_many([(o, t) for o, t in zip(out, tensors) if t.is_cuda and t.is_contiguous()])
+    return out
 
 
 @dataclass
diff --git a/temporally-consistent-stereo-matching_amd/tcs_mi355/s16.py b/temporally-consistent-stereo-matching_amd/tcs_mi355/s16.py
--- a/temporally-consistent-stereo-matching_amd/tcs_mi355/s16.py
+++ b/temporally-consistent-stereo-matching_amd/tcs_mi355/s16.py
@@ -2,7 +2,7 @@
 
 import ctypes as C
 from dataclasses import dataclass
-from typing import Dict, Optional, Sequence
+from typing import Dict, List, Optional, Sequence
 
 import torch
 
@@ -108,6 +108,23 @@
         raise ValueError("to_s16: `out` has another shape")
     nv.check(nv.lib().tcs_s16_from_f32(nv.ptr(x, "x"), B, C_, H, W, out.ptr(), out.G, int(group_offset), nv.stream()), "tcs_s16_from_f32")
     return out
+
+
+def to_s16_many(xs: Sequence[torch.Tensor], outs: Sequence[S16]) -> List[S16]:
+    if len(xs) != len(outs):
+        raise ValueError("to_s16_many: one `out` per tensor")
+    descs = []
+    for x, o in zip(xs, outs):
+        if x.ndim != 4:
+            raise ValueError("to_s16_many expects [B,C,H,W] tensors")
+        B, C_, H, W = (int(v) for v in x.shape)
+        if (o.B, o.H, o.W) != (B, H, W):
+            raise ValueError("to_s16_many: an `out` has another shape")
+        descs.append(nv.S16FromF32Desc(nv.ptr(x, "x"), B, C_, H, W, o.ptr(), o.G, 0))
+    for i in range(0, len(descs), nv.S16_FROM_F32_MANY):
+        part = descs[i:i + nv.S16_FROM_F32_MANY]
+        nv.check(nv.lib().tcs_s16_from_f32_many((nv.S16FromF32Desc * len(part))(*part), len(part), nv.stream()), "tcs_s16_from_f32_many")
+    return list(outs)
 
 
 def from_s16(s: S16, C_: Optional[int] = None, group_offset: int = 0, out: Optional[torch.Tensor] = None) -> torch.Tensor:
```

Result: no change. 37.72 (-0.2%).
